# pminervini/hyperopt

Hardware: AMD Instinct MI355X
Metric: EI candidates scored/sec (x components) (higher is better)
Workload: dtype f64 (log-sum-exp: fp64 accumulation, fp32 exp2 of the shifted term, its argument from an fp32 block-local quadratic (mode 3); quantized: fp64 erf); 1 GPU; config 4: 100-D uniform space, 1e4-trial history, 1e7 candidates/suggest (lpdf roofline stress); parallelism=single

## Files before the change

hyperopt_amd/_engine.py:

```python
from __future__ import annotations

import ctypes as C
import os
import threading

import numpy as np

_HERE = os.path.dirname(os.path.abspath(__file__))
LIB_PATH = os.environ.get('TPE_ENGINE_LIB', os.path.join(_HERE, 'libtpe_engine.so'))

TPE_OK = 0
TPE_E_INVALID = -1
TPE_E_BOUNDS = -2
TPE_E_NEGATIVE = -3
TPE_E_NOMEM = -4
TPE_E_HIP = -5
TPE_E_NODEVICE = -6
TPE_E_INDEX = -7

GMM, LGMM, CAT = 0, 1, 2
HAS_LOW, HAS_HIGH, HAS_Q, PCHOICE = 1, 2, 4, 8
OBS_IDENT, OBS_LOG, OBS_LOG_CLIP_EXPLOW, OBS_LOG_CLIP_EPS = 0, 1, 2, 3
KIND_NAMES = ('lse_gmm', 'lse_lgmm', 'erf_gmm', 'erf_lgmm', 'categorical')

EXPORTS = (
    'tpe_version', 'tpe_device_count', 'tpe_create', 'tpe_destroy', 'tpe_last_error',
    'tpe_synchronize', 'tpe_split', 'tpe_parzen_fit', 'tpe_categorical_posterior',
    'tpe_lpdf', 'tpe_score', 'tpe_sample', 'tpe_plan_create', 'tpe_plan_destroy',
    'tpe_plan_num_levels', 'tpe_plan_set_history', 'tpe_plan_fit', 'tpe_plan_get_mixture',
    'tpe_plan_get_table',
    'tpe_plan_suggest', 'tpe_plan_suggest_shard', 'tpe_plan_merge', 'tpe_plan_score_candidates', 'tpe_plan_last_stats',
    'tpe_plan_profile', 'tpe_plan_profile_read', 'tpe_microbench', 'tpe_plan_get_results',
    'tpe_plan_results_device', 'tpe_plan_census', 'tpe_plan_fit_suggest',
    'tpe_plan_set_lattice', 'tpe_plan_update_history', 'tpe_plan_set_prune',
    'tpe_plan_sample_prior', 'tpe_plan_score_candidates_sorted', 'tpe_plan_census_n',
    'tpe_plan_tie_counts', 'tpe_plan_tab_wmax', 'tpe_plan_anneal', 'tpe_plan_anneal_trace',
    'tpe_plan_set_anneal_order', 'tpe_plan_tab_bound', 'tpe_plan_tab_hot',
    'tpe_plan_tab_panels', 'tpe_plan_tab_cert', 'tpe_plan_tie_list',
    'tpe_plan_cand_dump', 'tpe_plan_draw_screen_stats', 'tpe_plan_score_points',
    'tpe_plan_sample_points', 'tpe_plan_topk_points', 'tpe_plan_gather_points',
    'tpe_plan_joint_fit', 'tpe_plan_joint_get_mixture', 'tpe_plan_joint_score_points',
    'tpe_plan_joint_sides', 'tpe_plan_joint_sample_points', 'tpe_math_probe',
    'tpe_plan_group_info', 'tpe_plan_group_fit', 'tpe_plan_group_get_mixture',
    'tpe_plan_group_score_points', 'tpe_plan_group_sides', 'tpe_plan_group_sample_points',
    'tpe_plan_group_batch_points',
    'tpe_plan_set_objectives', 'tpe_plan_pareto_get', 'tpe_plan_pareto_shape',
    'tpe_plan_set_hv', 'tpe_plan_hv_get',
)

BATCH_MAX = 1024
MAX_OBJ = 8

SHARD_ALIGN = 8192


class EngineUnavailable(RuntimeError):
    """The HIP engine library or an MI355X (gfx950) device is not available."""


class EngineError(RuntimeError):
    pass


class TpeHp(C.Structure):
    _fields_ = [('family', C.c_int32), ('flags', C.c_uint32), ('obs_transform', C.c_int32),
                ('upper', C.c_int32), ('prior_mu', C.c_double), ('prior_sigma', C.c_double),
                ('low', C.c_double), ('high', C.c_double), ('q', C.c_double),
                ('cond_begin', C.c_int32), ('cond_count', C.c_int32),
                ('pprior_begin', C.c_int64)]


class TpeSpace(C.Structure):
    _fields_ = [('n_hp', C.c_int32), ('hp', C.POINTER(TpeHp)), ('n_cond', C.c_int32),
                ('cond_parent', C.POINTER(C.c_int32)), ('cond_branch', C.POINTER(C.c_int32)),
                ('n_pprior', C.c_int64), ('pprior', C.POINTER(C.c_double))]


RESULT_DTYPE = np.dtype([('score', '<f8'), ('value', '<f8'), ('index', '<i8'),
                         ('active', '<i4'), ('pad', '<i4')])
ANNEAL_TRACE_DTYPE = np.dtype([('row', '<i4'), ('rank', '<i4'), ('u', '<f8', (4,))])

_D = C.POINTER(C.c_double)
_lib = None
_lib_lock = threading.Lock()


def _share_hip_runtime():
    if os.environ.get('TPE_ENGINE_HIP_RUNTIME', '') == 'system':
        return
    import importlib.util
    try:
        spec = importlib.util.find_spec('torch')
    except (ImportError, ValueError):
        spec = None
    if spec is None or not spec.origin:
        return
    hip = os.path.join(os.path.dirname(spec.origin), 'lib', 'libamdhip64.so')
    if os.path.exists(hip):
        C.CDLL(hip, mode=C.RTLD_GLOBAL)


def load_library(path: str = LIB_PATH):
    global _lib
    with _lib_lock:
        if _lib is not None:
            return _lib
        if not os.path.exists(path):
            raise EngineUnavailable(
                'libtpe_engine.so not found at %s: build it with `make -C '
                'hyperopt_amd/csrc` or __graft_entry__.build()' % path)
        _share_hip_runtime()
        lib = C.CDLL(path)
        vp, i32, i64, u32, u64, dbl = C.c_void_p, C.c_int32, C.c_int64, C.c_uint32, C.c_uint64, C.c_double
        sig = {
            'tpe_version': (C.c_char_p, []),
            'tpe_device_count': (C.c_int, [C.POINTER(i32)]),
            'tpe_create': (C.c_int, [i32, C.POINTER(vp)]),
            'tpe_destroy': (C.c_int, [vp]),
            'tpe_last_error': (C.c_char_p, [vp]),
            'tpe_synchronize': (C.c_int, [vp]),
            'tpe_split': (C.c_int, [vp, _D, i64, dbl, i32, C.POINTER(C.c_uint8)]),
            'tpe_parzen_fit': (C.c_int, [vp, _D, i64, dbl, dbl, dbl, i32, _D, _D, _D]),
            'tpe_categorical_posterior': (C.c_int, [vp, C.POINTER(i64), i64, i32, dbl, _D, i32, _D]),
            'tpe_lpdf': (C.c_int, [vp, i32, _D, i64, _D, _D, _D, i64, dbl, dbl, dbl, u32, _D]),
            'tpe_score': (C.c_int, [vp, i32, _D, i64, _D, _D, _D, i64, _D, _D, _D, i64,
                                    dbl, dbl, dbl, u32, _D, _D, C.POINTER(i64), _D]),
            'tpe_sample': (C.c_int, [vp, i32, _D, _D, _D, i64, dbl, dbl, dbl, u32, u64, u64,
                                     i64, i64, _D]),
            'tpe_plan_create': (C.c_int, [vp, C.POINTER(TpeSpace), i64, C.POINTER(vp)]),
            'tpe_plan_destroy': (C.c_int, [vp]),
            'tpe_plan_num_levels': (C.c_int, [vp, C.POINTER(i32)]),
            'tpe_plan_set_history': (C.c_int, [vp, vp, vp, vp, i64, i32, vp]),
            'tpe_plan_update_history': (C.c_int, [vp, i64, i64, i64, vp, vp, i64, i64, vp, i32,
                                                  vp]),
            'tpe_plan_fit': (C.c_int, [vp, dbl, i32, dbl, i32, vp]),
            'tpe_plan_get_mixture': (C.c_int, [vp, i32, i32, _D, _D, _D, i64, C.POINTER(i64)]),
            'tpe_plan_get_table': (C.c_int, [vp, i32, i32, i32, vp, i64, C.POINTER(i64)]),
            'tpe_plan_suggest': (C.c_int, [vp, C.POINTER(u64), i64, i64, i64, i32, vp, i32, vp]),
            'tpe_plan_suggest_shard': (C.c_int, [vp, C.POINTER(u64), i64, i64, i64, i64, i32, vp,
                                                 i32, vp]),
            'tpe_plan_fit_suggest': (C.c_int, [vp, dbl, i32, dbl, i32, C.POINTER(u64), i64, i64,
                                               vp, i32, vp]),
            'tpe_plan_merge': (C.c_int, [vp, vp, i32, i32, vp, i32, vp]),
            'tpe_plan_score_candidates': (C.c_int, [vp, i32, _D, i64, _D, _D, C.POINTER(i64), _D]),
            'tpe_plan_score_candidates_sorted': (C.c_int, [vp, i32, i32, _D, i64, _D, _D,
                                                           C.POINTER(i64), _D]),
            'tpe_plan_score_points': (C.c_int, [vp, vp, i64, i64, vp, vp, vp, i32, vp]),
            'tpe_plan_sample_points': (C.c_int, [vp, u64, i64, i64, i64, vp, vp, vp, vp, i32, vp]),
            'tpe_plan_topk_points': (C.c_int, [vp, vp, vp, i64, i32, vp, i32, vp]),
            'tpe_plan_joint_fit': (C.c_int, [vp, vp]),
            'tpe_plan_joint_get_mixture': (C.c_int, [vp, i32, i32, _D, _D, _D, vp, i64,
                                                     C.POINTER(i64)]),
            'tpe_plan_joint_score_points': (C.c_int, [vp, vp, i64, i64, vp, vp, vp, vp, i32, vp]),
            'tpe_plan_joint_sides': (C.c_int, [vp, vp, vp, i64]),
            'tpe_plan_joint_sample_points': (C.c_int, [vp, u64, i64, i64, i64, vp, vp, vp, vp, vp,
                                                       vp, i32, vp]),
            'tpe_plan_group_info': (C.c_int, [vp, vp, C.POINTER(i32)]),
            'tpe_plan_group_fit': (C.c_int, [vp, vp]),
            'tpe_plan_group_get_mixture': (C.c_int, [vp, i32, i32, i32, _D, _D, _D, vp, i64,
                                                     C.POINTER(i64)]),
            'tpe_plan_group_score_points': (C.c_int, [vp, vp, i64, i64, vp, vp, vp, i32, vp]),
            'tpe_plan_group_sides': (C.c_int, [vp, i32, vp, vp, i64]),
            'tpe_plan_group_sample_points': (C.c_int, [vp, u64, i64, i64, i64, vp, vp, vp, vp, vp,
                                                       i32, vp]),
            'tpe_plan_group_batch_points': (C.c_int, [vp, vp, i64, i64, vp, i32, vp, vp, vp, i32,
                                                      vp]),
            'tpe_plan_gather_points': (C.c_int, [vp, vp, i64, vp, i32, vp, i32, vp]),
            'tpe_plan_set_objectives': (C.c_int, [vp, vp, i32, i64, i64, i64, i32, vp]),
            'tpe_plan_pareto_get': (C.c_int, [vp, vp, vp, vp, i64]),
            'tpe_plan_pareto_shape': (C.c_int, [vp, i64, i32, i64, C.POINTER(i64)]),
            'tpe_plan_set_hv': (C.c_int, [vp, i32, vp, i32, i32, i32, C.c_uint64, i32]),
            'tpe_plan_hv_get': (C.c_int, [vp, vp, vp, vp, C.POINTER(i32), i32]),
            'tpe_plan_last_stats': (C.c_int, [vp, _D, _D]),
            'tpe_plan_profile': (C.c_int, [vp, i32]),
            'tpe_plan_profile_read': (C.c_int, [vp, i32, _D, C.POINTER(i64), _D]),
            'tpe_microbench': (C.c_int, [vp, i32, _D]),
            'tpe_math_probe': (C.c_int, [vp, i32, _D, i64, _D]),
            'tpe_plan_get_results': (C.c_int, [vp, vp, i32, vp]),
            'tpe_plan_results_device': (vp, [vp]),
            'tpe_plan_census': (C.c_int, [vp, i32, C.POINTER(i64)]),
            'tpe_plan_census_n': (C.c_int, [vp, i32, C.POINTER(i64), i32]),
            'tpe_plan_tie_counts': (C.c_int, [vp, i32, vp]),
            'tpe_plan_tab_wmax': (C.c_int, [vp, i32, vp]),
            'tpe_plan_tab_bound': (C.c_int, [vp, i32, vp]),
            'tpe_plan_tab_hot': (C.c_int, [vp, i32, vp]),
            'tpe_plan_tab_panels': (C.c_int, [vp, i32, i32, vp, vp, vp, vp]),
            'tpe_plan_tab_cert': (C.c_int, [vp, i32, i32, vp]),
            'tpe_plan_tie_list': (C.c_int, [vp, i32, i32, vp]),
            'tpe_plan_cand_dump': (C.c_int64, [vp, i32, i32, vp, vp]),
            'tpe_plan_draw_screen_stats': (C.c_int, [vp, vp]),
            'tpe_plan_set_lattice': (C.c_int, [vp, i32]),
            'tpe_plan_set_prune': (C.c_int, [vp, i32]),
            'tpe_plan_sample_prior': (C.c_int, [vp, C.POINTER(u64), i64, vp, i32, vp]),
            'tpe_plan_anneal': (C.c_int, [vp, dbl, dbl, C.POINTER(u64), i64, vp, i32, vp]),
            'tpe_plan_anneal_trace': (C.c_int, [vp, i32, vp]),
            'tpe_plan_set_anneal_order': (C.c_int, [vp, C.POINTER(i32), i32]),
        }
        for name, (res, args) in sig.items():
            fn = getattr(lib, name)
            fn.restype = res
            fn.argtypes = args
        _lib = lib
        return lib


def _seeds(seeds):
    seeds = [int(x) & (2 ** 64 - 1) for x in np.atleast_1d(np.asarray(seeds, dtype=object))]
    return np.fromiter(seeds, dtype=np.uint64, count=len(seeds))


def _dp(a):
    return None if a is None else a.ctypes.data_as(_D)


def _f64(a):
    return np.ascontiguousarray(a, dtype=np.float64)


class Engine(object):

    def __init__(self, device: int = 0):
        self.lib = load_library()
        n = C.c_int32(0)
        self.lib.tpe_device_count(C.byref(n))
        if n.value <= 0:
            raise EngineUnavailable('no HIP device visible (TPE engine needs an MI355X)')
        h = C.c_void_p()
        rc = self.lib.tpe_create(int(device), C.byref(h))
        if rc != TPE_OK:
            raise EngineUnavailable('tpe_create(%d) failed (%d): not a gfx950 device?' % (device, rc))
        self.h = h
        self.device = device
        self.lock = threading.RLock()

    def close(self):
        if getattr(self, 'h', None):
            self.lib.tpe_destroy(self.h)
            self.h = None

    def __del__(self):
        try:
            self.close()
        except Exception:
            pass

    def check(self, rc):
        if rc == TPE_OK:
            return
        msg = (self.lib.tpe_last_error(self.h) or b'').decode()
        if rc == TPE_E_BOUNDS:
            raise ValueError('low >= high', msg)
        if rc == TPE_E_NEGATIVE:
            raise ValueError('negative arg to lognormal_cdf', msg)
        if rc == TPE_E_INDEX:
            raise IndexError(msg)
        if rc == TPE_E_INVALID:
            raise ValueError(msg)
        raise EngineError('TPE engine error %d: %s' % (rc, msg))

    def synchronize(self):
        with self.lock:
            self.check(self.lib.tpe_synchronize(self.h))

    def microbench(self, which):
        r = C.c_double(0)
        with self.lock:
            self.check(self.lib.tpe_microbench(self.h, int(which), C.byref(r)))
        return r.value

    def math_probe(self, which, x):
        xa = _f64(x)
        xs = xa.ravel()
        out = np.empty(xs.size)
# ... 741 lines not shown
        with e.lock:
            e.check(e.lib.tpe_plan_census_n(self.p, int(bool(enable)), out, int(n)))
        return tuple(int(v) for v in out[:n])

    def tie_counts(self, n_suggest):
        e = self.engine
        out = np.empty((int(n_suggest), self.n_hp), dtype=np.int32)
        with e.lock:
            e.check(e.lib.tpe_plan_tie_counts(self.p, int(n_suggest), out.ctypes.data))
        return out

    def tab_wmax(self, n_suggest):
        e = self.engine
        with e.lock:
            w = e.lib.tpe_plan_tab_wmax(self.p, int(n_suggest), None)
            e.check(min(w, 0))
            out = np.empty((int(n_suggest), self.n_hp, w), dtype=np.float64)
            e.check(e.lib.tpe_plan_tab_wmax(self.p, int(n_suggest), out.ctypes.data))
        return out

    def tab_bound(self, hp):
        e = self.engine
        with e.lock:
            n = e.lib.tpe_plan_tab_bound(self.p, int(hp), None)
            e.check(min(n, 0))
            out = np.empty(n, dtype=np.float64)
            e.check(e.lib.tpe_plan_tab_bound(self.p, int(hp), out.ctypes.data))
        return out

    def tab_panels(self, hp, side):
        e = self.engine
        y_lo, inv_w, ncert = C.c_double(), C.c_double(), C.c_int32()
        buf = np.zeros((64, 144), dtype=np.uint8)
        with e.lock:
            n = e.lib.tpe_plan_tab_panels(self.p, int(hp), int(side), C.addressof(y_lo),
                                          C.addressof(inv_w), C.addressof(ncert), buf.ctypes.data)
            e.check(min(n, 0))
        return dict(y_lo=y_lo.value, inv_w=inv_w.value, P=int(n), ncert=int(ncert.value),
                    panels=buf[:n].copy())

    def tab_cert(self, hp, side):
        e = self.engine
        out = np.zeros((64, 3), dtype=np.float64)
        with e.lock:
            n = e.lib.tpe_plan_tab_cert(self.p, int(hp), int(side), out.ctypes.data)
            e.check(min(n, 0))
        return out[:n].copy()

    def tie_list(self, s, hp):
        e = self.engine
        with e.lock:
            n = e.lib.tpe_plan_tie_list(self.p, int(s), int(hp), None)
            e.check(min(n, 0))
            out = np.empty(n, dtype=np.int32)
            if n:
                e.check(min(e.lib.tpe_plan_tie_list(self.p, int(s), int(hp), out.ctypes.data), 0))
        return out

    def tab_hot(self, n_suggest):
        e = self.engine
        out = np.empty((int(n_suggest), self.n_hp, 18), dtype=np.float64)
        with e.lock:
            e.check(e.lib.tpe_plan_tab_hot(self.p, int(n_suggest), out.ctypes.data))
        return out

    def cand_dump(self, s, hp):
        e = self.engine
        with e.lock:
            n = e.lib.tpe_plan_cand_dump(self.p, int(s), int(hp), None, None)
            e.check(int(min(n, 0)))
            vals = np.empty(n, dtype=np.float64)
            pos = np.empty(n, dtype=np.int32)
            e.check(int(min(e.lib.tpe_plan_cand_dump(self.p, int(s), int(hp), vals.ctypes.data,
                                                     pos.ctypes.data), 0)))
        return vals, pos

    def draw_screen_stats(self):
        e = self.engine
        out = np.zeros(3, dtype=np.int64)
        with e.lock:
            e.check(e.lib.tpe_plan_draw_screen_stats(self.p, out.ctypes.data))
        return int(out[0]), int(out[1]), int(out[2])

    def last_stats(self):
        e = self.engine
        ms, pairs = C.c_double(0), C.c_double(0)
        with e.lock:
            e.check(e.lib.tpe_plan_last_stats(self.p, C.byref(ms), C.byref(pairs)))
        return ms.value, pairs.value


_default = {}
_default_lock = threading.Lock()


def default_engine(device: int | None = None) -> Engine:
    if device is None:
        device = int(os.environ.get('LOCAL_RANK', '0'))
    with _default_lock:
        eng = _default.get(device)
        if eng is None:
            eng = Engine(device)
            _default[device] = eng
        return eng
```

hyperopt_amd/csrc/tpe_engine.hip:

```cpp
#include <hip/hip_runtime.h>

#include <algorithm>
#include <cmath>
#include <cstdlib>
#include <cstdio>
#include <cstring>
#include <string>
#include <vector>

#include "tpe_anneal.hpp"
#include "tpe_group_plan.hpp"
#include "tpe_internal.hpp"
#include "tpe_level_plan.hpp"
#include "tpe_pareto_plan.hpp"
#include "tpe_hv_plan.hpp"
#include "tpe_switches.hpp"

using namespace tpe;
static_assert(sizeof(AnnealTrace) == sizeof(tpe_anneal_trace), "layout");

struct tpe_engine {
  int32_t device = 0;
  hipStream_t stream = nullptr;
  static constexpr int kAux = 4;
  hipStream_t aux[kAux] = {};
  std::string err;
  tpe_plan *op = nullptr;
};

struct tpe_plan : PlanShape {
  tpe_engine *eng = nullptr;
  int32_t P = 0;
  int64_t ncap = 0;
  int32_t last_nb = -1;
  std::vector<double> pprior;
  std::vector<int32_t> level_off;
  tpe_hp *d_hps = nullptr;
  int32_t *d_cp = nullptr, *d_cb = nullptr, *d_level_hps = nullptr, *d_all_hps = nullptr;
  int32_t *d_level_off = nullptr;
  double *d_pprior = nullptr;
  double *d_losses = nullptr, *d_vals = nullptr;
  uint8_t *d_active = nullptr, *d_below = nullptr;
  double *d_mw = nullptr, *d_mmu = nullptr, *d_msig = nullptr, *d_scratch = nullptr;
  unsigned char *d_sortbuf = nullptr;
  int64_t scap = 0;
  MixInfo *d_info = nullptr;
  Coef *d_coef = nullptr;
  Coef32 *d_coef32 = nullptr;
  CoefM *d_coefm = nullptr;
  CoefM8 *d_coefm8 = nullptr;
  float4 *d_coefe = nullptr;
  CoefM8 *d_coefmh = nullptr;
  TabHdr *d_tab_hdr = nullptr;
  TabPanel *d_tab = nullptr;
  double *d_tab_max = nullptr;
  double *d_tab_wmax = nullptr;
  int32_t *d_tie_list = nullptr;
  int32_t *d_tie_cnt = nullptr;
  int32_t tab_pstride = 0;
  double *d_tab_bound = nullptr;
  double *d_tab_terms = nullptr;
  double *d_tab_cert = nullptr;
  TabHot *d_tab_hot = nullptr;
  DrawZone *d_draw_zone = nullptr;
  unsigned long long *d_screen_stats = nullptr;
  bool tab_built = false;
  bool graph_tab = false;
  int64_t n = 0;
  int64_t s_cap = 0;
  Partial *d_results = nullptr;
  tpe_result *h_results = nullptr;
  size_t h_results_cap = 0;
  uint64_t *h_flag = nullptr;
  uint64_t seq = 0;
  bool pub_fired = false;
  uint64_t *d_seeds = nullptr;
  Partial *d_partial = nullptr;
  size_t partial_cap = 0;
  unsigned long long *d_census = nullptr;
  bool census = false;
  uint32_t *d_ticket = nullptr;
  std::vector<uint64_t> h_seeds;
  bool has_erf = false;
  LatInfo *d_lat_info = nullptr;
  double2 *d_lat = nullptr;
  bool lattice_on = true;
  int32_t prune_mode = 3;
  hipEvent_t ev_fork = nullptr, ev_join[8] = {};
  double *d_ext = nullptr, *d_lb = nullptr, *d_la = nullptr;
  size_t ext_cap = 0;
  double *d_pt_vals = nullptr, *d_pt_terms = nullptr, *d_pt_total = nullptr;
  uint8_t *d_pt_act = nullptr;
  int32_t *d_pt_idx = nullptr;
  uint32_t *d_pt_count = nullptr;
  size_t pt_cap = 0;
  void *d_pt_tab = nullptr;
  void *d_tk = nullptr;
  int32_t *d_tk_idx = nullptr;
  double *d_cand = nullptr;
  int32_t *d_cpos = nullptr;
  size_t cand_cap = 0;
  std::vector<JointDim> jdims;
  std::vector<int32_t> jdim_of_hp;
  int32_t j_slots = 0;
  int64_t j_nopt = 0;
  bool joint_ok = false;
  int32_t jK[2] = {0, 0};
  double fit_pw = 1.0;
  int32_t fit_lf = 0;
  JointDim *d_jdims = nullptr;
  int32_t *d_jdim_of_hp = nullptr, *d_jrows = nullptr, *d_jcount = nullptr, *d_jcomp = nullptr;
  JointSide *d_jside = nullptr;
  uint64_t *d_jkeys = nullptr;
  double *d_jw = nullptr, *d_jcw = nullptr, *d_jcmu = nullptr, *d_jcsig = nullptr;
  double *d_jtab = nullptr, *d_joptlog = nullptr, *d_jpick = nullptr, *d_joptcdf = nullptr;
  size_t joptcdf_cap = 0;
  void *d_jdraw = nullptr;
  double *d_jsides = nullptr, *d_jjoint = nullptr;
  size_t jpt_cap = 0;
  int64_t jpt_m = 0;
  GroupPartition gpart;
  GroupLayout glay;
  bool group_ready = false, group_ok = false;
  int32_t gkb_max = 0;
  JointDim *d_gdims = nullptr;
  GroupDesc *d_ggroups = nullptr;
  int32_t *d_gdim_of_hp = nullptr, *d_ggroup_of_hp = nullptr, *d_grows = nullptr;
  int32_t *d_gcount = nullptr, *d_gcomp = nullptr;
  JointSide *d_gside = nullptr;
  uint64_t *d_gkeys = nullptr;
  double *d_gw = nullptr, *d_gcw = nullptr, *d_gcmu = nullptr, *d_gcsig = nullptr;
  double *d_gtab = nullptr, *d_goptlog = nullptr, *d_gpick = nullptr, *d_goptcdf = nullptr;
  size_t goptcdf_cap = 0;
  void *d_gdraw = nullptr;
  double *d_gsides = nullptr, *d_gjoint = nullptr;
  size_t gpt_cap = 0;
  int64_t gpt_m = 0;
  double *d_bt_ja = nullptr, *d_bt_score = nullptr, *d_bt_gain = nullptr, *d_bt_trace = nullptr;
  uint8_t *d_bt_gact = nullptr, *d_bt_state = nullptr;
  void *d_bt_slot = nullptr, *d_bt_rec = nullptr;
  int32_t *d_bt_idx = nullptr;
  size_t bt_cap = 0, bt_trace_cap = 0;
  int64_t bt_m = -1;
  hipEvent_t ev0 = nullptr, ev1 = nullptr;
  struct Prof {
    std::vector<hipEvent_t> a, b;
    std::vector<double> pairs;
    int64_t n = 0;
  };
  Prof prof[KIND_CAT + 1];
  int32_t prof_cap = 0;
  bool timed = false;
  bool evs = false;
  int64_t last_ncand = 0, last_nsug = 0;
  int32_t last_level = -1;
  int64_t dump_cn = 0, dump_sstride = 0, dump_nsug = 0;
  int32_t dump_level = -1;
  struct StepKey {
    double prior_weight = 0;
    int32_t lf = 0;
    void *stream = nullptr;
    StepShape shape;
    bool operator==(const StepKey &o) const {
      return prior_weight == o.prior_weight && lf == o.lf && stream == o.stream &&
             shape == o.shape;
    }
  };
  StepKey graph_key, pending_key;
  bool graph_ok = false, pending = false;
  int32_t mom_w = 0;
  bool mom_h = false;
// ... 31 lines not shown
  bool hv_last_exact = false;
  hipGraph_t graph = nullptr;
  hipGraphExec_t graph_exec = nullptr;
  std::vector<hipGraphNode_t> fit_nodes, draw_nodes;
  std::vector<hipKernelNodeParams> fit_params, draw_params;
  std::vector<FitArgs> fit_args0;
  std::vector<ScoreArgs> draw_args0;
};

namespace {

#define CKH(expr)                                                        \
  do {                                                                   \
    hipError_t e_ = (expr);                                              \
    if (e_ != hipSuccess) {                                              \
      return fail(h, TPE_E_HIP, std::string(#expr) + ": " + hipGetErrorString(e_)); \
    }                                                                    \
  } while (0)

int fail(tpe_engine *h, int code, const std::string &msg) {
  if (h) h->err = msg;
  return code;
}

template <typename T>
hipError_t dalloc(T **p, size_t count) {
  *p = nullptr;
  if (count == 0) count = 1;
  return hipMalloc((void **)p, count * sizeof(T));
}

void dfree(void *p) {
  if (p) (void)hipFree(p);
}

void graph_reset(tpe_plan *p) {
  if (p->graph_exec) (void)hipGraphExecDestroy(p->graph_exec);
  if (p->graph) (void)hipGraphDestroy(p->graph);
  p->graph_exec = nullptr;
  p->graph = nullptr;
  p->graph_ok = p->pending = false;
  p->fit_nodes.clear(); p->draw_nodes.clear();
  p->fit_params.clear(); p->draw_params.clear();
  p->fit_args0.clear(); p->draw_args0.clear();
}

hipStream_t pick_stream(tpe_engine *h, void *s) {
  return s ? (hipStream_t)s : h->stream;
}

void plan_free_buffers(tpe_plan *p) {
  void *bufs[] = {p->d_an_keys, p->d_an_idx, p->d_an_T, p->d_an_hporder, p->d_an_trace,
                  p->d_hps, p->d_cp, p->d_cb, p->d_level_hps, p->d_all_hps, p->d_pprior,
                  p->d_level_off,
                  p->d_losses, p->d_vals, p->d_active, p->d_below, p->d_mw, p->d_mmu,
                  p->d_msig, p->d_scratch, p->d_info, p->d_coef, p->d_results, p->d_seeds,
                  p->d_partial, p->d_ext, p->d_lb, p->d_la, p->d_cand, p->d_cpos,
                  p->d_ticket, p->d_sortbuf, p->d_census, p->d_lat_info, p->d_lat, p->d_coef32, p->d_coefm,
                  p->d_coefm8, p->d_coefe, p->d_coefmh, p->d_tab_hdr, p->d_tab,
                  p->d_tab_max, p->d_tab_wmax, p->d_tie_list, p->d_tie_cnt, p->d_tab_bound,
                  p->d_tab_terms, p->d_tab_cert,
                  p->d_tab_hot, p->d_draw_zone, p->d_screen_stats, p->d_pt_vals, p->d_pt_terms,
                  p->d_pt_total, p->d_pt_act, p->d_pt_idx, p->d_pt_count, p->d_pt_tab, p->d_tk,
                  p->d_tk_idx, p->d_jdims, p->d_jdim_of_hp, p->d_jrows, p->d_jcount, p->d_jcomp,
                  p->d_jside, p->d_jkeys, p->d_jw, p->d_jcw, p->d_jcmu, p->d_jcsig, p->d_jtab,
                  p->d_joptlog, p->d_jpick, p->d_joptcdf, p->d_jdraw, p->d_jsides, p->d_jjoint,
                  p->d_gdims, p->d_ggroups, p->d_gdim_of_hp, p->d_ggroup_of_hp, p->d_grows,
                  p->d_gcount, p->d_gcomp, p->d_gside, p->d_gkeys, p->d_gw, p->d_gcw, p->d_gcmu,
                  p->d_gcsig, p->d_gtab, p->d_goptlog, p->d_gpick, p->d_goptcdf, p->d_gdraw,
                  p->d_gsides, p->d_gjoint, p->d_bt_ja, p->d_bt_score, p->d_bt_gain,
                  p->d_bt_trace, p->d_bt_gact, p->d_bt_state, p->d_bt_slot, p->d_bt_rec,
                  p->d_bt_idx, p->d_obj, p->d_pcount, p->d_hv_i32, p->d_hv_f64, p->d_hv_alive,
                  p->d_hv_u};
  for (void *b : bufs) dfree(b);
  if (p->h_results) (void)hipHostFree(p->h_results);
  p->h_results = nullptr;
  p->h_results_cap = 0;
  if (p->h_flag) (void)hipHostFree(p->h_flag);
  p->h_flag = nullptr;
  if (p->ev0) (void)hipEventDestroy(p->ev0);
  if (p->ev1) (void)hipEventDestroy(p->ev1);
  if (p->ev_fork) (void)hipEventDestroy(p->ev_fork);
  for (auto e : p->ev_join) if (e) (void)hipEventDestroy(e);
  for (auto &pr : p->prof) {
    for (auto e : pr.a) (void)hipEventDestroy(e);
    for (auto e : pr.b) (void)hipEventDestroy(e);
    pr.a.clear(); pr.b.clear(); pr.pairs.clear(); pr.n = 0;
  }
}

int validate_space(tpe_engine *h, const tpe_space *sp) {
  if (!sp || sp->n_hp <= 0 || !sp->hp) return fail(h, TPE_E_INVALID, "empty space");
  for (int i = 0; i < sp->n_hp; ++i) {
    const tpe_hp &x = sp->hp[i];
    if (x.family < TPE_GMM || x.family > TPE_CAT)
      return fail(h, TPE_E_INVALID, "hp " + std::to_string(i) + ": bad family");
    if (x.family == TPE_CAT && x.upper <= 0)
      return fail(h, TPE_E_INVALID, "hp " + std::to_string(i) + ": categorical upper <= 0");
    if (x.family != TPE_CAT) {
      const bool hl = x.flags & TPE_HAS_LOW, hh = x.flags & TPE_HAS_HIGH;
      if (hl != hh)
        return fail(h, TPE_E_INVALID, "hp " + std::to_string(i) + ": one-sided truncation");
      if (hl && !(x.low < x.high))
        return fail(h, TPE_E_BOUNDS, "low >= high");
      if (!(x.prior_sigma > 0))
        return fail(h, TPE_E_INVALID, "hp " + std::to_string(i) + ": prior_sigma <= 0");
    }
    if (x.cond_count < 0 || x.cond_begin < 0 || x.cond_begin + x.cond_count > sp->n_cond)
      return fail(h, TPE_E_INVALID, "hp " + std::to_string(i) + ": bad condition range");
    for (int c = 0; c < x.cond_count; ++c) {
      const int par = sp->cond_parent[x.cond_begin + c];
      if (par < 0 || par >= sp->n_hp || par == i)
        return fail(h, TPE_E_INVALID, "hp " + std::to_string(i) + ": bad condition parent");
    }
    if ((x.flags & TPE_PCHOICE) &&
        (x.pprior_begin < 0 || x.pprior_begin + x.upper > sp->n_pprior))
      return fail(h, TPE_E_INVALID, "hp " + std::to_string(i) + ": bad pchoice prior");
  }
  return TPE_OK;
}

LatInfo lattice_of(const tpe_hp &x) {
  LatInfo L{0, 0, 0, 0};
  const int k = score_kind(x);
  if (k != KIND_ERF_G && k != KIND_ERF_L) return L;
  if (!(x.flags & TPE_HAS_LOW) || !(x.flags & TPE_HAS_HIGH) || !(x.q > 0.0)) return L;
  double lo = x.low, hi = x.high;
  if (k == KIND_ERF_L) {
    lo = std::exp(lo);
    hi = std::exp(hi);
  }
  const double a = std::rint(lo / x.q) - 2.0, b = std::rint(hi / x.q) + 2.0;
  if (!(std::fabs(a) < 1e15 && std::fabs(b) < 1e15) || b - a + 1.0 > (double)kLatMaxR)
    return L;
  L.j0 = (int64_t)a;
  L.R = (int32_t)(b - a + 1.0);
  return L;
}

int compute_levels(tpe_engine *h, tpe_plan *p) {
  std::vector<int> lev(p->P, -1);
  for (int iter = 0; iter <= p->P; ++iter) {
    bool changed = false;
    for (int i = 0; i < p->P; ++i) {
      const tpe_hp &x = p->hps[i];
      int l = 0;
      bool ready = true;
      for (int c = 0; c < x.cond_count; ++c) {
        const int par = p->cond_parent[x.cond_begin + c];
        if (lev[par] < 0) { ready = false; break; }
        l = std::max(l, lev[par] + 1);
      }
      if (ready && lev[i] != l) { lev[i] = l; changed = true; }
    }
    if (!changed) break;
  }
  int nl = 0;
  for (int i = 0; i < p->P; ++i) {
    if (lev[i] < 0 || lev[i] > p->P) return fail(h, TPE_E_INVALID, "cyclic conditions");
    nl = std::max(nl, lev[i] + 1);
  }
  p->levels.assign(nl, {});
  for (int lat : {1, 0})
    for (int kind : {KIND_ERF_L, KIND_ERF_G})
      for (int i = 0; i < p->P; ++i)
        if (score_kind(p->hps[i]) == kind && (lattice_of(p->hps[i]).R > 0) == (lat == 1))
// ... 10 lines not shown
int plan_build(tpe_engine *h, const tpe_space *sp, int64_t max_trials, tpe_plan *p) {
  int rc = validate_space(h, sp);
  if (rc) return rc;
  if (max_trials < 0) return fail(h, TPE_E_INVALID, "max_trials < 0");
  p->eng = h;
  p->P = sp->n_hp;

  p->hps.assign(sp->hp, sp->hp + sp->n_hp);
  p->cond_parent.assign(sp->cond_parent, sp->cond_parent + sp->n_cond);
  p->cond_branch.assign(sp->cond_branch, sp->cond_branch + sp->n_cond);
  p->pprior.assign(sp->pprior, sp->pprior + sp->n_pprior);
  rc = compute_levels(h, p);
  if (rc) return rc;
  p->ncap = std::max<int64_t>(max_trials, 1);
  int64_t kcap = p->ncap + 1;
  for (const auto &x : p->hps)
    if (x.family == TPE_CAT) kcap = std::max<int64_t>(kcap, x.upper);
  kcap = (kcap + kCoefBlock - 1) / kCoefBlock * kCoefBlock;
  p->kcap = kcap;
  for (const auto &x : p->hps) {
    const int k = score_kind(x);
    if (k == KIND_ERF_G || k == KIND_ERF_L) p->has_erf = true;
  }
  const int64_t slots = 2 * (int64_t)p->P;
  p->lat.assign(p->P, LatInfo{0, 0, 0, 0});
  int64_t lat_total = 0;
  for (int i = 0; i < p->P; ++i) {
    p->lat[i] = lattice_of(p->hps[i]);
    p->lat[i].off = lat_total;
    lat_total += p->lat[i].R;
  }
  CKH(hipSetDevice(h->device));
  CKH(dalloc(&p->d_lat_info, p->P));
  CKH(dalloc(&p->d_lat, std::max<int64_t>(1, lat_total)));
  CKH(dalloc(&p->d_hps, p->P));
  CKH(dalloc(&p->d_cp, p->cond_parent.size()));
  CKH(dalloc(&p->d_cb, p->cond_branch.size()));
  CKH(dalloc(&p->d_pprior, p->pprior.size()));
  CKH(dalloc(&p->d_level_hps, p->P));
  CKH(dalloc(&p->d_all_hps, p->P));
  CKH(dalloc(&p->d_level_off, p->level_off.size()));
  CKH(dalloc(&p->d_losses, p->ncap));
  CKH(dalloc(&p->d_vals, (size_t)p->ncap * p->P));
  CKH(dalloc(&p->d_active, (size_t)p->ncap * p->P));
  CKH(dalloc(&p->d_below, p->ncap));
  CKH(dalloc(&p->d_mw, (size_t)slots * kcap));
  CKH(dalloc(&p->d_mmu, (size_t)slots * kcap));
  CKH(dalloc(&p->d_msig, (size_t)slots * kcap));
  CKH(dalloc(&p->d_scratch, (size_t)slots * kcap));
  p->scap = p->ncap + 1;
  CKH(dalloc(&p->d_sortbuf, (size_t)slots * 16 * p->scap));
  CKH(dalloc(&p->d_info, slots));
  CKH(dalloc(&p->d_census, kCensus));
  CKH(hipMemset(p->d_census, 0, kCensus * sizeof(unsigned long long)));
  CKH(dalloc(&p->d_coef, (size_t)slots * kcap));
  CKH(dalloc(&p->d_coef32, (size_t)slots * (kcap / kCoefBlock)));
  CKH(dalloc(&p->d_coefm, (size_t)slots * mom_stride(kcap)));
  CKH(dalloc(&p->d_coefm8, (size_t)slots * (kcap / kCoefBlock)));
  CKH(dalloc(&p->d_coefe, (size_t)slots * (kcap / kCoefBlock)));
  CKH(dalloc(&p->d_coefmh, (size_t)slots * mom_stride(kcap)));
  CKH(dalloc(&p->d_tab_hdr, (size_t)slots));
  CKH(hipMemset(p->d_tab_hdr, 0, (size_t)slots * sizeof(TabHdr)));
  CKH(dalloc(&p->d_tab, (size_t)slots * kTabMaxPanels));
  CKH(dalloc(&p->d_tab_bound, (size_t)p->P * kBndCells));
  if (switches().table_lean) CKH(dalloc(&p->d_tab_terms, table_terms_doubles(p->P, kcap)));
  p->act_frac.assign(p->P, 1.0);
  for (const auto &lv : p->levels)
    for (int i : lv) {
      const tpe_hp &x = p->hps[i];
      if (x.cond_count == 0) continue;
      double f = 0.0;
      for (int c = 0; c < x.cond_count; ++c) {
        const int par = p->cond_parent[x.cond_begin + c];
        const tpe_hp &y = p->hps[par];
        f += p->act_frac[par] / (y.family == TPE_CAT ? std::max(1, (int)y.upper) : 1);
      }
      p->act_frac[i] = std::min(1.0, f);
    }
  p->finish();
  CKH(hipEventCreate(&p->ev0));
  CKH(hipEventCreate(&p->ev1));
  CKH(hipEventCreateWithFlags(&p->ev_fork, hipEventDisableTiming));
  for (auto &e : p->ev_join) CKH(hipEventCreateWithFlags(&e, hipEventDisableTiming));
  std::vector<int32_t> lh;
  for (auto &l : p->levels) lh.insert(lh.end(), l.begin(), l.end());
  std::vector<int32_t> all(p->P);
  for (int i = 0; i < p->P; ++i) all[i] = i;
  hipStream_t st = h->stream;
  CKH(hipMemcpyAsync(p->d_hps, p->hps.data(), p->P * sizeof(tpe_hp), hipMemcpyHostToDevice, st));
  CKH(hipMemcpyAsync(p->d_lat_info, p->lat.data(), p->P * sizeof(LatInfo), hipMemcpyHostToDevice,
                     st));
  if (!p->cond_parent.empty()) {
    CKH(hipMemcpyAsync(p->d_cp, p->cond_parent.data(), p->cond_parent.size() * 4, hipMemcpyHostToDevice, st));
    CKH(hipMemcpyAsync(p->d_cb, p->cond_branch.data(), p->cond_branch.size() * 4, hipMemcpyHostToDevice, st));
  }
  if (!p->pprior.empty())
    CKH(hipMemcpyAsync(p->d_pprior, p->pprior.data(), p->pprior.size() * 8, hipMemcpyHostToDevice, st));
  CKH(hipMemcpyAsync(p->d_level_hps, lh.data(), lh.size() * 4, hipMemcpyHostToDevice, st));
  CKH(hipMemcpyAsync(p->d_all_hps, all.data(), all.size() * 4, hipMemcpyHostToDevice, st));
  CKH(hipMemcpyAsync(p->d_level_off, p->level_off.data(), p->level_off.size() * 4,
                     hipMemcpyHostToDevice, st));
  CKH(hipMemsetAsync(p->d_info, 0, slots * sizeof(MixInfo), st));
  CKH(hipStreamSynchronize(st));
  return TPE_OK;
}

int ensure_suggest_state(tpe_engine *h, tpe_plan *p, int64_t n_sug, size_t partials) {
  if (n_sug > p->s_cap || partials > p->partial_cap) graph_reset(p);
  if (n_sug > p->s_cap) {
    dfree(p->d_results);
    dfree(p->d_seeds);
    dfree(p->d_ticket);
    p->d_results = nullptr;
    p->d_seeds = nullptr;
    p->d_ticket = nullptr;
    CKH(dalloc(&p->d_results, (size_t)n_sug * p->P));
    CKH(dalloc(&p->d_seeds, n_sug));
    CKH(dalloc(&p->d_ticket, (size_t)n_sug * p->P + 1));
    CKH(hipMemset(p->d_ticket, 0, ((size_t)n_sug * p->P + 1) * sizeof(uint32_t)));
    dfree(p->d_tab_max);
    p->d_tab_max = nullptr;
    CKH(dalloc(&p->d_tab_max, (size_t)n_sug * p->P));
    dfree(p->d_tie_cnt);
    p->d_tie_cnt = nullptr;
    CKH(dalloc(&p->d_tie_cnt, (size_t)n_sug * p->P));
    CKH(hipMemset(p->d_tie_cnt, 0xff, (size_t)n_sug * p->P * sizeof(int32_t)));
    dfree(p->d_tab_hot);
    p->d_tab_hot = nullptr;
    CKH(dalloc(&p->d_tab_hot, (size_t)n_sug * p->P));
    dfree(p->d_draw_zone);
    p->d_draw_zone = nullptr;
    CKH(dalloc(&p->d_draw_zone, (size_t)n_sug * p->P));
    if (!p->d_screen_stats) {
      CKH(dalloc(&p->d_screen_stats, 2));
      CKH(hipMemset(p->d_screen_stats, 0, 2 * sizeof(unsigned long long)));
    }
    p->s_cap = n_sug;
  }
  if (partials > p->partial_cap) {
    dfree(p->d_partial);
    p->d_partial = nullptr;
    CKH(dalloc(&p->d_partial, partials));
    dfree(p->d_tab_wmax);
    p->d_tab_wmax = nullptr;
    CKH(dalloc(&p->d_tab_wmax, partials * 8));
    CKH(hipMemset(p->d_tab_wmax, 0xff, partials * 8 * sizeof(double)));
    dfree(p->d_tie_list);
    p->d_tie_list = nullptr;
    CKH(dalloc(&p->d_tie_list, partials * 8));
    p->partial_cap = partials;
  }
  return TPE_OK;
}

int ensure_ext(tpe_engine *h, tpe_plan *p, size_t n) {
  if (n > p->ext_cap) {
    dfree(p->d_ext); dfree(p->d_lb); dfree(p->d_la);
    p->d_ext = p->d_lb = p->d_la = nullptr;
    CKH(dalloc(&p->d_ext, n));
    CKH(dalloc(&p->d_lb, n));
    CKH(dalloc(&p->d_la, n));
    p->ext_cap = n;
  }
  return TPE_OK;
}

// ... 113 lines not shown
  a.n_below = n_below;
  a.lf = lf;
  a.prior_weight = prior_weight;
  a.pprior = p->d_pprior;
  a.mw = p->d_mw;
  a.mmu = p->d_mmu;
  a.msig = p->d_msig;
  a.info = p->d_info;
  a.coef = p->d_coef;
  a.coef32 = p->d_coef32;
  a.coefm = p->mom_w == 16 ? p->d_coefm : nullptr;
  a.coefm8 = p->mom_w == 8 ? p->d_coefm8 : nullptr;
  a.coefmh = p->mom_h ? p->d_coefmh : nullptr;
  a.coefe = p->d_coefe;
  a.kcap = p->kcap;
  a.ob = p->d_scratch;
  a.tmp = p->d_scratch;
  a.sortbuf = p->d_sortbuf;
  a.scap = p->scap;
  return a;
}

int flush_patch(tpe_engine *h, tpe_plan *p, hipStream_t st) {
  if (!p->has_pend) return TPE_OK;
  p->has_pend = false;
  CKH(launch_hist_patch(p->pend, p->d_vals, p->d_active, p->d_losses, st));
  return TPE_OK;
}
int fit_launch(tpe_engine *h, tpe_plan *p, const FitArgs &a, int32_t n_hp, hipStream_t st) {
  CKH(launch_fit(a, n_hp, st, p->has_pend ? &p->pend : nullptr));
  p->has_pend = false;
  return TPE_OK;
}

int table_build(tpe_engine *h, tpe_plan *p, hipStream_t st) {
  if (p->tab_built) return TPE_OK;
  CKH(launch_table_build(p->d_hps, p->P, p->d_info, p->d_coef, p->kcap, p->d_tab_hdr, p->d_tab,
                         p->census ? p->d_census : nullptr, st,
                         switches().table_prefilter ? p->d_tab_bound : nullptr, p->d_tab_terms,
                         p->d_tab_cert));
  p->tab_built = true;
  return TPE_OK;
}

int score_launch(tpe_engine *h, tpe_plan *p, ScoreArgs a, bool has_erf, int64_t cn,
                 hipStream_t sg, bool record, int classes = 7) {
  tpe_plan::Prof *pr = nullptr;
  if (record && p->prof_cap > 0) {
    pr = &p->prof[0];
    if (pr->n >= p->prof_cap) pr = nullptr;
  }
  if (pr) CKH(hipEventRecord(pr->a[pr->n], sg));
  if (a.tab_on == 1 && (classes & 1)) {
    const int rc = table_build(h, p, sg);
    if (rc) return rc;
    p->tab_pstride = a.pstride;
  }
  CKH(launch_score(a, has_erf, sg, switches().side_streams ? h->aux[1] : nullptr, p->ev_join[1],
                   p->ev_join[2], classes));
  if (pr) {
    CKH(hipEventRecord(pr->b[pr->n], sg));
    pr->pairs[pr->n] = (double)cn * (double)a.n_suggest;
    pr->n++;
  }
  return TPE_OK;
}

StepShape step_shape(const tpe_plan *p, int64_t n_sug, int64_t n_cand, int64_t cand_begin,
                     int64_t n_total, int32_t last_nb, const FitVariant &f) {
  StepShape s;
  s.n_sug = n_sug;
  s.n_cand = n_cand;
  s.cand_begin = cand_begin;
  s.n_total = n_total;
  s.below = below_class(last_nb >= 0 ? (int64_t)last_nb + 1 : p->kcap);
  s.fit = f;
  s.prune_mode = p->prune_mode;
  s.lattice_on = p->lattice_on;
  s.screen_run = step_screen_run(switches());
  s.screen_halves = step_screen_halves(switches());
  s.screen_tail = (int32_t)switches().draw_screen_tail;
  s.screen_pool = switches().draw_screen_pool;
  s.table_lean = switches().table_lean;
  return s;
}

int run_level(tpe_engine *h, tpe_plan *p, int level, const StepShape &s, hipStream_t st) {
  const LevelPlan lp = plan_level(*p, switches(), s, level);
  const int64_t n_sug = s.n_sug;
  const int32_t n_level = lp.n_level, n_lat = lp.n_lat;
  const int32_t *lvl = p->d_level_hps + p->level_off[level];
  if (lp.empty) {
    if (n_level > 0) CKH(launch_merge(lvl, n_level, (int32_t)n_sug, p->P, 0, nullptr, p->d_results, st));
    return TPE_OK;
  }
  ScoreArgs la = base_args(p, n_sug);
  la.level_hps = lvl;
  la.n_slots = n_level;
  la.slot_rows = lp.slot_rows;
  la.compact = lp.compact ? 1 : 0;
  auto lat_bracket = [&](hipStream_t sl, auto launch) -> int {
    tpe_plan::Prof *pr = nullptr;
    if (p->prof_cap > 0 && p->prof[1].n < p->prof_cap) pr = &p->prof[1];
    if (pr) CKH(hipEventRecord(pr->a[pr->n], sl));
    CKH(launch());
    if (pr) {
      CKH(hipEventRecord(pr->b[pr->n], sl));
      pr->pairs[pr->n] = (double)level;
      pr->n++;
    }
    return TPE_OK;
  };
  auto lattice = [&](hipStream_t sl) -> int {
    return lat_bracket(sl, [&] {
      return launch_lattice(la, p->levels[level].data(), p->hps.data(), p->lat.data(), n_lat,
                            p->d_lat, sl, lp.lat_rows);
    });
  };
  const bool lat_side = lp.lat == LatRun::Side;
  bool lat_pending = lp.lat == LatRun::Deferred;
  if (lp.lat == LatRun::InOrder || lat_side) {
    hipStream_t sl = st;
    if (lat_side) {
      sl = h->aux[0];
      CKH(hipEventRecord(p->ev_fork, st));
      CKH(hipStreamWaitEvent(sl, p->ev_fork, 0));
    }
    const int lrc = lattice(sl);
    if (lat_side) {
      const hipError_t e1 = hipEventRecord(p->ev_join[0], sl);
      if (lrc) {
        if (e1 == hipSuccess) (void)hipStreamWaitEvent(st, p->ev_join[0], 0);
        return lrc;
      }
      if (e1 != hipSuccess) return fail(h, TPE_E_HIP, "lattice side stream join event");
    } else if (lrc) {
      return lrc;
    }
  }
  bool joined = !lat_side;
  auto chunks = [&]() -> int {
  for (const ChunkPlan &c : lp.chunks) {
    const int64_t cn = c.cn;
    if (c.grid.pstride < 0) return fail(h, TPE_E_INVALID, "level slots not grouped by lpdf kind");
    int rc = ensure_suggest_state(h, p, n_sug, (size_t)n_sug * p->P * c.grid.pstride);
    if (rc) return rc;
    rc = ensure_cand(h, p, (size_t)std::max<int64_t>(1, n_sug * n_level * cn));
    if (rc) return rc;
    ScoreArgs a = base_args(p, n_sug);
    copy_groups(a, c.grid);
    a.compact = lp.compact ? 1 : 0;
    a.cand = p->d_cand;
    a.cand_sstride = (int64_t)n_level * cn;
    a.n_cand = cn;
    a.cand_begin = s.cand_begin + c.c0;
    a.accumulate = c.accumulate ? 1 : 0;
    a.level_hps = lvl;
    a.n_slots = n_level;
    a.slot_rows = lp.slot_rows;
    a.cand_slot0 = 0;
    for (int i = 0; i < kInlineSeeds && i < n_sug; ++i) a.seed_inline[i] = p->h_seeds[i];
    a.n_inline_seeds = (int32_t)std::min<int64_t>(n_sug, kInlineSeeds);
    a.lse_pos = c.lse_pos;
    a.sort_log2 = c.sort_log2;
    a.lookup_draw = c.lookup_draw;
    a.lse_prune = c.lse_prune;
    a.lse_shift_min = lp.lse_shift_min;
    a.lse_f32 = c.lse_f32;
    a.tab_on = c.tab_on;
    a.tab_pref = c.tab_pref ? 1 : 0;
    if (c.lk_fork) {
// ... 816 lines not shown
  if (mi.K > cap) return fail(h, TPE_E_INVALID, "capacity too small");
  if (w) CKH(hipMemcpy(w, p->d_mw + slot * p->kcap, mi.K * 8, hipMemcpyDeviceToHost));
  if (mu) CKH(hipMemcpy(mu, p->d_mmu + slot * p->kcap, mi.K * 8, hipMemcpyDeviceToHost));
  if (sigma) CKH(hipMemcpy(sigma, p->d_msig + slot * p->kcap, mi.K * 8, hipMemcpyDeviceToHost));
  return TPE_OK;
}

int tpe_plan_get_table(tpe_plan_t p, int32_t hp, int32_t side, int32_t which, void *out,
                       int64_t cap_bytes, int64_t *bytes) {
  if (!p || !bytes) return TPE_E_INVALID;
  tpe_engine *h = p->eng;
  if (hp < 0 || hp >= p->P || side < 0 || side > 1 || which < 0 || which > 4)
    return fail(h, TPE_E_INVALID, "bad hp/side/table");
  CKH(hipSetDevice(h->device));
  CKH(hipDeviceSynchronize());
  const int64_t slot = 2 * (int64_t)hp + side;
  const void *src = nullptr;
  if (which == 0) {
    *bytes = p->kcap * (int64_t)sizeof(Coef);
    src = p->d_coef + slot * p->kcap;
  } else if (which == 1) {
    *bytes = p->kcap / kCoefBlock * (int64_t)sizeof(Coef32);
    src = p->d_coef32 + slot * (p->kcap / kCoefBlock);
  } else if (which == 2) {
    *bytes = mom_stride(p->kcap) * (int64_t)sizeof(CoefM);
    src = p->d_coefm + slot * mom_stride(p->kcap);
  } else if (which == 3) {
    *bytes = p->kcap / kCoefBlock * (int64_t)sizeof(CoefM8);
    src = p->d_coefm8 + slot * (p->kcap / kCoefBlock);
  } else {
    *bytes = mom_stride(p->kcap) * (int64_t)sizeof(CoefM8);
    src = p->d_coefmh + slot * mom_stride(p->kcap);
  }
  if (!out) return TPE_OK;
  if (*bytes > cap_bytes) return fail(h, TPE_E_INVALID, "capacity too small");
  CKH(hipMemcpy(out, src, (size_t)*bytes, hipMemcpyDeviceToHost));
  return TPE_OK;
}

int tpe_plan_suggest(tpe_plan_t p, const uint64_t *seeds, int64_t n_sug, int64_t n_cand,
                     int64_t cand_begin, int32_t level, tpe_result *out, int32_t out_on_device,
                     void *stream) {
  return tpe_plan_suggest_shard(p, seeds, n_sug, cand_begin + n_cand, cand_begin, n_cand, level,
                                out, out_on_device, stream);
}

int tpe_plan_suggest_shard(tpe_plan_t p, const uint64_t *seeds, int64_t n_sug, int64_t n_total,
                           int64_t cand_begin, int64_t n_cand, int32_t level, tpe_result *out,
                           int32_t out_on_device, void *stream) {
  if (!p) return TPE_E_INVALID;
  tpe_engine *h = p->eng;
  if (n_sug <= 0 || n_cand < 0 || cand_begin < 0 || !seeds || n_total < cand_begin + n_cand)
    return fail(h, TPE_E_INVALID, "bad args");
  if (level >= (int32_t)p->levels.size()) return fail(h, TPE_E_INVALID, "bad level");
  CKH(hipSetDevice(h->device));
  hipStream_t st = pick_stream(h, stream);
  int rc = ensure_suggest_state(h, p, n_sug, 1);
  if (rc) return rc;
  p->h_seeds.assign(seeds, seeds + n_sug);
  if (n_sug > kInlineSeeds)
    CKH(hipMemcpyAsync(p->d_seeds, seeds, n_sug * 8, hipMemcpyHostToDevice, st));
  if (p->prof_cap > 0) CKH(hipEventRecord(p->ev0, st));
  const int l0 = level < 0 ? 0 : level;
  const int l1 = level < 0 ? (int)p->levels.size() : level + 1;
  const StepShape s = step_shape(p, n_sug, n_cand, cand_begin, n_total, p->last_nb,
                                 FitVariant{fit_small(p->n), p->mom_w, p->mom_h});
  for (int l = l0; l < l1; ++l) {
    rc = run_level(h, p, l, s, st);
    if (rc) return rc;
  }
  if (p->prof_cap > 0) CKH(hipEventRecord(p->ev1, st));
  p->timed = true;
  p->evs = p->prof_cap > 0;
  p->last_ncand = n_cand;
  p->last_nsug = n_sug;
  p->last_level = level;
  return copy_results(h, p, n_sug, out, out_on_device, st);
}

namespace {

int enqueue_step(tpe_engine *h, tpe_plan *p, int32_t nb, double prior_weight, int32_t lf,
                 const StepShape &s, hipStream_t st) {
  {
    const int rc = fit_launch(h, p, fit_args(p, nb, prior_weight, lf, s.fit), p->P, st);
    if (rc) return rc;
  }
  p->last_nb = nb;
  for (int l = 0; l < (int)p->levels.size(); ++l) {
    const int rc = run_level(h, p, l, s, st);
    if (rc) return rc;
  }
  return TPE_OK;
}

int capture_step(tpe_engine *h, tpe_plan *p, int32_t nb, double prior_weight, int32_t lf,
                 const StepShape &s, hipStream_t st) {
  graph_reset(p);
  CKH(hipStreamBeginCapture(st, hipStreamCaptureModeThreadLocal));
  const int rc = enqueue_step(h, p, nb, prior_weight, lf, s, st);
  hipGraph_t g = nullptr;
  const hipError_t ec = hipStreamEndCapture(st, &g);
  if (rc || ec != hipSuccess || !g) {
    if (g) (void)hipGraphDestroy(g);
    return rc ? rc : fail(h, TPE_E_HIP, "graph capture failed");
  }
  p->graph = g;
  p->graph_mom_w = p->mom_w;
  p->graph_mom_h = p->mom_h;
  p->graph_tab = p->tab_built;
  CKH(hipGraphInstantiate(&p->graph_exec, g, nullptr, nullptr, 0));
  size_t nn = 0;
  CKH(hipGraphGetNodes(g, nullptr, &nn));
  std::vector<hipGraphNode_t> nodes(nn);
  CKH(hipGraphGetNodes(g, nodes.data(), &nn));
  for (hipGraphNode_t nd : nodes) {
    hipGraphNodeType ty;
    CKH(hipGraphNodeGetType(nd, &ty));
    if (ty != hipGraphNodeTypeKernel) continue;
    hipKernelNodeParams kp{};
    CKH(hipGraphKernelNodeGetParams(nd, &kp));
    if (kp.func == fit_kernel_fn(true) || kp.func == fit_kernel_fn(false)) {
      p->fit_nodes.push_back(nd);
      p->fit_params.push_back(kp);
      p->fit_args0.push_back(*static_cast<const FitArgs *>(kp.kernelParams[0]));
    } else if (is_draw_kernel_fn(kp.func) || kp.func == lattice_draw_kernel_fn()) {
      p->draw_nodes.push_back(nd);
      p->draw_params.push_back(kp);
      p->draw_args0.push_back(*static_cast<const ScoreArgs *>(kp.kernelParams[0]));
    }
  }
  if (p->fit_nodes.size() != 1) {
    graph_reset(p);
    return fail(h, TPE_E_HIP, "graph capture: fit node not found");
  }
  p->graph_ok = true;
  return TPE_OK;
}

int launch_step(tpe_engine *h, tpe_plan *p, int32_t nb, const uint64_t *seeds, int64_t n_sug,
                hipStream_t st) {
  for (size_t i = 0; i < p->fit_nodes.size(); ++i) {
    FitArgs fa = p->fit_args0[i];
    fa.n = p->n;
    fa.n_below = nb;
    HistPatch none{};
    void *args[2] = {&fa, &none};
    hipKernelNodeParams kp = p->fit_params[i];
    kp.kernelParams = args;
    kp.extra = nullptr;
    CKH(hipGraphExecKernelNodeSetParams(p->graph_exec, p->fit_nodes[i], &kp));
  }
  for (size_t i = 0; i < p->draw_nodes.size(); ++i) {
    ScoreArgs da = p->draw_args0[i];
    for (int64_t j = 0; j < n_sug; ++j) da.seed_inline[j] = seeds[j];
    da.n_inline_seeds = (int32_t)n_sug;
    hipKernelNodeParams kp = p->draw_params[i];
    LatJobs jobs{};
    double2 *lat_out = nullptr;
    int32_t *pos_out = nullptr;
    const DrawZone *zones = nullptr;
    unsigned long long *stats = nullptr;
    int32_t run = 0;
    void *args[5] = {&da, &jobs, &lat_out, &stats, &run};
    if (kp.func == lattice_draw_kernel_fn()) {
      jobs = *static_cast<const LatJobs *>(kp.kernelParams[1]);
// ... 1410 lines not shown
  TabHdr th[2];
  CKH(hipMemcpyAsync(th, p->d_tab_hdr + 2 * (int64_t)hp, sizeof(th), hipMemcpyDeviceToHost,
                     h->stream));
  CKH(hipStreamSynchronize(h->stream));
  for (const TabHdr &t : th)
    if (!(t.P > 0 && t.ncert == (uint32_t)t.P))
      return fail(h, TPE_E_INVALID, "Chebyshev table not certified");
  CKH(hipMemcpy(out, p->d_tab_bound + (int64_t)hp * kBndCells, kBndCells * sizeof(double),
                hipMemcpyDeviceToHost));
  return TPE_OK;
}

static int tab_header(tpe_plan *p, int32_t hp, int32_t side, TabHdr *th) {
  tpe_engine *h = p->eng;
  if (hp < 0 || hp >= p->P || side < 0 || side > 1) return fail(h, TPE_E_INVALID, "bad args");
  if (!table_hp(p->hps[hp])) return fail(h, TPE_E_INVALID, "hp has no Chebyshev table");
  CKH(hipSetDevice(h->device));
  CKH(hipDeviceSynchronize());
  const int rc = table_build(h, p, h->stream);
  if (rc) return rc;
  CKH(hipMemcpyAsync(th, p->d_tab_hdr + 2 * (int64_t)hp + side, sizeof(*th), hipMemcpyDeviceToHost,
                     h->stream));
  CKH(hipStreamSynchronize(h->stream));
  if (th->P < 0 || th->P > kTabMaxPanels) return fail(h, TPE_E_HIP, "table header out of range");
  return TPE_OK;
}

int tpe_plan_tab_panels(tpe_plan_t p, int32_t hp, int32_t side, double *y_lo, double *inv_w,
                        int32_t *ncert, void *panels) {
  if (!p) return TPE_E_INVALID;
  tpe_engine *h = p->eng;
  TabHdr th;
  const int rc = tab_header(p, hp, side, &th);
  if (rc) return rc;
  if (y_lo) *y_lo = th.y_lo;
  if (inv_w) *inv_w = th.inv_w;
  if (ncert) *ncert = (int32_t)th.ncert;
  if (panels && th.P > 0)
    CKH(hipMemcpy(panels, p->d_tab + (2 * (int64_t)hp + side) * kTabMaxPanels,
                  (size_t)th.P * sizeof(TabPanel), hipMemcpyDeviceToHost));
  return th.P;
}

int tpe_plan_tab_cert(tpe_plan_t p, int32_t hp, int32_t side, double *out) {
  if (!p) return TPE_E_INVALID;
  tpe_engine *h = p->eng;
  if (!p->d_tab_cert) {
    CKH(hipSetDevice(h->device));
    CKH(hipDeviceSynchronize());
    graph_reset(p);
    const size_t n = (size_t)2 * p->P * kTabMaxPanels * 3;
    CKH(dalloc(&p->d_tab_cert, n));
    CKH(hipMemset(p->d_tab_cert, 0xff, n * sizeof(double)));
    p->tab_built = false;
  }
  TabHdr th;
  const int rc = tab_header(p, hp, side, &th);
  if (rc) return rc;
  if (out && th.P > 0)
    CKH(hipMemcpy(out, p->d_tab_cert + (2 * (int64_t)hp + side) * kTabMaxPanels * 3,
                  (size_t)th.P * 3 * sizeof(double), hipMemcpyDeviceToHost));
  return th.P;
}

int tpe_plan_tie_list(tpe_plan_t p, int32_t s, int32_t hp, int32_t *out) {
  if (!p) return TPE_E_INVALID;
  tpe_engine *h = p->eng;
  if (hp < 0 || hp >= p->P || s < 0 || s >= p->s_cap || p->tab_pstride <= 0 ||
      ((size_t)s * p->P + hp + 1) * p->tab_pstride > p->partial_cap)
    return fail(h, TPE_E_INVALID, "hp / suggestion not of the last launch that took the tables");
  CKH(hipSetDevice(h->device));
  CKH(hipDeviceSynchronize());
  int32_t n = 0;
  CKH(hipMemcpy(&n, p->d_tie_cnt + (int64_t)s * p->P + hp, sizeof(n), hipMemcpyDeviceToHost));
  const int64_t row = (int64_t)p->tab_pstride * 8;
  if (n < 0) return 0;
  if (n > row) return fail(h, TPE_E_HIP, "tie count out of range");
  if (out && n > 0)
    CKH(hipMemcpy(out, p->d_tie_list + ((int64_t)s * p->P + hp) * row, (size_t)n * sizeof(int32_t),
                  hipMemcpyDeviceToHost));
  return n;
}

int tpe_plan_draw_screen_stats(tpe_plan_t p, int64_t *out) {
  if (!p || !out) return TPE_E_INVALID;
  tpe_engine *h = p->eng;
  out[0] = out[1] = out[2] = 0;
  if (!p->d_screen_stats) return TPE_OK;
  CKH(hipSetDevice(h->device));
  CKH(hipDeviceSynchronize());
  unsigned long long v[2];
  CKH(hipMemcpy(v, p->d_screen_stats, sizeof(v), hipMemcpyDeviceToHost));
  CKH(hipMemset(p->d_screen_stats, 0, sizeof(v)));
  out[0] = (int64_t)(v[0] >> 40);
  out[1] = (int64_t)v[1];
  out[2] = (int64_t)(v[0] & ((1ull << 40) - 1));
  return TPE_OK;
}

int tpe_plan_tab_hot(tpe_plan_t p, int32_t n_suggest, double *out) {
  static_assert(sizeof(TabHot) == (2 + 2 * kHotIv) * sizeof(double), "y_lo, y_hi, lo[], hi[]");
  if (!p || !out || n_suggest < 0) return TPE_E_INVALID;
  tpe_engine *h = p->eng;
  if (n_suggest > p->s_cap) return fail(h, TPE_E_INVALID, "more suggestions than the last call's");
  CKH(hipSetDevice(h->device));
  CKH(hipDeviceSynchronize());
  if (n_suggest > 0)
    CKH(hipMemcpy(out, p->d_tab_hot, (size_t)n_suggest * p->P * sizeof(TabHot),
                  hipMemcpyDeviceToHost));
  return TPE_OK;
}

int tpe_plan_sample_prior(tpe_plan_t p, const uint64_t *seeds, int64_t n_sug, tpe_result *out,
                          int32_t out_on_device, void *stream) {
  if (!p) return TPE_E_INVALID;
  tpe_engine *h = p->eng;
  if (n_sug <= 0 || !seeds) return fail(h, TPE_E_INVALID, "bad args");
  CKH(hipSetDevice(h->device));
  hipStream_t st = pick_stream(h, stream);
  int rc = ensure_suggest_state(h, p, n_sug, 1);
  if (rc) return rc;
  CKH(hipMemcpyAsync(p->d_seeds, seeds, n_sug * 8, hipMemcpyHostToDevice, st));
  PriorArgs a{};
  a.hps = p->d_hps;
  a.n_hp = p->P;
  a.n_levels = (int32_t)p->levels.size();
  a.level_hps = p->d_level_hps;
  a.level_off = p->d_level_off;
  a.cond_parent = p->d_cp;
  a.cond_branch = p->d_cb;
  a.pprior = p->d_pprior;
  a.seeds = p->d_seeds;
  a.results = p->d_results;
  CKH(launch_prior(a, (int32_t)n_sug, st));
  p->last_nsug = n_sug;
  if (!out_on_device) {
    rc = copy_results(h, p, n_sug, out, 0, st);
    if (rc) return rc;
    return TPE_OK;
  }
  return copy_results(h, p, n_sug, out, out_on_device, st);
}

int tpe_plan_set_anneal_order(tpe_plan_t p, const int32_t *hp_order, int32_t n_hp) {
  if (!p) return TPE_E_INVALID;
  tpe_engine *h = p->eng;
  if (!hp_order || n_hp != p->P) return fail(h, TPE_E_INVALID, "anneal order: one entry per hp");
  std::vector<int32_t> pos(p->P, -1);
  for (int k = 0; k < n_hp; ++k) {
    const int hp = hp_order[k];
    if (hp < 0 || hp >= p->P || pos[hp] >= 0)
      return fail(h, TPE_E_INVALID, "anneal order: not a permutation of the hps");
    pos[hp] = k;
  }
  for (int hp = 0; hp < p->P; ++hp) {
    const tpe_hp &x = p->hps[hp];
    for (int c = 0; c < x.cond_count; ++c)
      if (pos[p->cond_parent[x.cond_begin + c]] > pos[hp])
        return fail(h, TPE_E_INVALID, "anneal order: an hp before the choice that leads to it");
  }
  CKH(hipSetDevice(h->device));
  p->an_order = false;
  if (!p->d_an_hporder) CKH(dalloc(&p->d_an_hporder, p->P));
  CKH(hipDeviceSynchronize());
  CKH(hipMemcpy(p->d_an_hporder, hp_order, (size_t)n_hp * 4, hipMemcpyHostToDevice));
  p->an_order = true;
// ... 179 lines not shown
```

hyperopt_amd/csrc/tpe_fit.hip:

```cpp
#include <math.h>

#include "tpe_device.hpp"

#pragma clang fp contract(off)

namespace tpe {

#define NOINLINE __attribute__((noinline))

#ifdef TPE_STAMPS
__device__ unsigned long long g_stamps[512][48];
#define STAMP(ph)                                                             \
  do {                                                                        \
    if (threadIdx.x == 0 && blockIdx.z == 0)                                  \
      g_stamps[(2 * blockIdx.x + blockIdx.y) & 511][ph] = wall_clock64();     \
  } while (0)
#else
#define STAMP(ph) do {} while (0)
#endif

constexpr int kFitWaves = kFitThreads / 64;
constexpr int kSortCap = 10000;
constexpr int kMixLds = 4097;
constexpr int kMixStride = 4104;
// ... 863 lines not shown
  __syncthreads();
  uint32_t tot = 0, mine = 0;
#pragma unroll
  for (int w = 0; w < kFitWaves; ++w) {
    const uint32_t c = wc[w * kCatFastBins + lane];
    tot += c;
    mine += w < wv ? c : 0u;
  }
  const uint32_t start = wave_excl_scan_u32(tot);
  if (wv == 0 && lane < upper) {
    seg[2 * lane] = (int)start;
    seg[2 * lane + 1] = (int)(start + tot);
  }
  uint32_t run = start + mine;
  double *ws = reinterpret_cast<double *>(C.lds + kOffKeys);
  const LfRamp lr = lf_ramp(m, A.lf);
  const uint64_t lt = lane ? (~0ull >> (64 - lane)) : 0ull;
#pragma unroll
  for (int q = 0; q < kCatFastChunks; ++q) {
    if (q * 64 >= per) break;
    uint32_t rank = 0, inc = 0;
    for (int b = 0; b < upper; ++b) {
      const uint64_t bal = __ballot(kr[q] == b);
      if (kr[q] == b) rank = (uint32_t)__popcll(bal & lt);
      if (lane == b) inc = (uint32_t)__popcll(bal);
    }
    const uint32_t base = (uint32_t)__shfl((int)run, kr[q] < 0 ? 0 : kr[q], 64);
    if (kr[q] >= 0) ws[base + rank] = lf_weight(lr, (int64_t)(r0 + q * 64 + lane));
    run += inc;
  }
  __syncthreads();
  STAMP(41);
  categorical_tail(A, sm, H, slot, seg, ws);
}

__device__ __forceinline__ void categorical_tail(const FitArgs &A, FitShared &sm, const tpe_hp &H,
                                                 int64_t slot, const int *seg, const double *ws) {
  const int upper = H.upper;
  double *w = A.mw + slot * A.kcap, *mu = A.mmu + slot * A.kcap, *sg = A.msig + slot * A.kcap;
  for (int c = threadIdx.x; c < upper; c += blockDim.x) {
    double cnt = 0.0;
    const int r1 = seg[2 * c + 1];
    int r = seg[2 * c];
    for (; r + 8 <= r1; r += 8) {
      double wv[8];
#pragma unroll
      for (int u = 0; u < 8; ++u) wv[u] = ws[r + u];
#pragma unroll
      for (int u = 0; u < 8; ++u) cnt += wv[u];
    }
    for (; r < r1; ++r) cnt += ws[r];
    double pc;
    if (H.flags & TPE_PCHOICE)
      pc = cnt + (double)upper * (A.prior_weight * A.pprior[H.pprior_begin + c]);
    else
      pc = cnt + A.prior_weight;
    w[c] = pc;
  }
  __syncthreads();
  STAMP(5);
  const double tot = block_np_sum(w, upper, sm);
  for (int c = threadIdx.x; c < upper; c += blockDim.x) {
    w[c] = w[c] / tot;
    mu[c] = 0.0;
    sg[c] = 0.0;
  }
  __syncthreads();
  prep_slot(A.hps + slot / 2, slot, upper, w, mu, sg, A.info, A.coef, A.coef32, A.coefm, A.coefm8,
            A.coefe, A.kcap, A.tmp + slot * A.kcap, sm);
}

#ifndef TPE_FIT_REPS
#define TPE_FIT_REPS 1
#endif
template <bool SMALL>
__device__ __forceinline__ void fit_slot(const FitArgs &A, unsigned char *dyn_lds,
                                         FitShared &sm);

template <bool SMALL>
__global__ __launch_bounds__(kFitThreads) void k_fit(FitArgs A, HistPatch P) {
  extern __shared__ __attribute__((aligned(16))) unsigned char dyn_lds[];
  __shared__ FitShared sm;
  if (P.n_rows > 0 || P.n_loss > 0) {
    const int hp = blockIdx.x;
    double *vals = const_cast<double *>(A.vals);
    uint8_t *act = const_cast<uint8_t *>(A.active);
    double *losses = const_cast<double *>(A.losses);
    for (int r = threadIdx.x; r < (int)P.n_rows; r += blockDim.x) {
      vals[(int64_t)hp * P.ld + P.row0 + r] = P.vals[hp * (int)P.n_rows + r];
      act[(int64_t)hp * P.ld + P.row0 + r] = P.active[hp * (int)P.n_rows + r];
    }
    for (int i = threadIdx.x; i < (int)P.n_loss; i += blockDim.x) losses[P.loss0 + i] = P.losses[i];
    __threadfence_block();
    __syncthreads();
  }
  for (int rep = 0; rep < TPE_FIT_REPS; ++rep) {
    fit_slot<SMALL>(A, dyn_lds, sm);
    __syncthreads();
  }
}

template <bool SMALL>
__device__ __forceinline__ void fit_slot(const FitArgs &A, unsigned char *dyn_lds,
                                         FitShared &sm) {
  const int hp = blockIdx.x, side = blockIdx.y;
  const int64_t slot = 2 * (int64_t)hp + side;
  const tpe_hp H = A.hps[hp];
  FitCtx C;
  C.lds = dyn_lds;
  unsigned char *gsb = A.sortbuf + slot * 16 * A.scap;
  C.gkeys = reinterpret_cast<uint64_t *>(gsb);
  C.gpa = reinterpret_cast<uint32_t *>(gsb + 8 * A.scap);
  C.gpb = C.gpa + A.scap;
  STAMP(0);
#ifdef TPE_STAMPS
  const unsigned long long clk0 = clock64();
#endif
  const bool pre = SMALL || A.n <= kPreN;
  constexpr int PER = SMALL ? 1 : kGatherRows;
  const double *row = A.vals + (int64_t)hp * A.ld;
  const uint8_t *arow = A.active + (int64_t)hp * A.ld;
  double prv[PER];
  uint8_t pac[PER];
  if (pre) {
#pragma unroll
    for (int u = 0; u < PER; ++u) {
      const int64_t j = min<int64_t>((int64_t)u * kFitThreads + threadIdx.x, A.n - 1);
      pac[u] = j >= 0 ? arow[j] : 0;
      prv[u] = j >= 0 ? row[j] : 0.0;
    }
  }
  const Split t = compute_split<SMALL>(A, C, sm);
  __syncthreads();
  STAMP(1);

  const bool cat = H.family == TPE_CAT;
  double *ob = (SMALL || A.n <= kMergeMax)
                   ? reinterpret_cast<double *>(dyn_lds + kOffKeys + 8 * kMergeMax)
                   : A.ob + slot * A.kcap;
  uint64_t *lk = reinterpret_cast<uint64_t *>(dyn_lds + kOffKeys);
  const uint64_t *lkey = (SMALL || A.n <= kSortCap) ? lk : C.gkeys;
  int m = 0;
  const int lane = threadIdx.x & 63, wv = threadIdx.x >> 6;
  for (int64_t c0 = 0; c0 < A.n; c0 += PER * kFitThreads) {
    if (!pre) {
#pragma unroll
      for (int u = 0; u < PER; ++u) {
        const int64_t j = min<int64_t>(c0 + (int64_t)u * kFitThreads + threadIdx.x, A.n - 1);
        pac[u] = arow[j];
        prv[u] = row[j];
      }
    }
    uint32_t fm = 0u;
#pragma unroll
    for (int u = 0; u < PER; ++u) {
      const int64_t j = c0 + (int64_t)u * kFitThreads + threadIdx.x;
      const bool f = j < A.n && pac[u] && (is_below(t, lkey[j], (uint32_t)j) == (side == 0));
      fm |= f ? 1u << u : 0u;
      const uint64_t b = __ballot(f);
      if (lane == 0) sm.gcnt[u][wv] = (int)__popcll(b);
    }
    STAMP(35);
    __syncthreads();
    if (wv == 0) {
      constexpr int NE = PER * kFitWaves, E = (NE + 63) / 64;
      const int *gc = &sm.gcnt[0][0];
      int *gb = &sm.gbase[0][0];
      int c[E], loc = 0;
#pragma unroll
      for (int e = 0; e < E; ++e) {
        const int q = lane * E + e;
        c[e] = q < NE ? gc[q] : 0;
        loc += c[e];
      }
      int acc = wave_incl_scan(loc) - loc;
#pragma unroll
      for (int e = 0; e < E; ++e) {
        const int q = lane * E + e;
        if (q < NE) gb[q] = acc;
        acc += c[e];
      }
    }
    __syncthreads();
    STAMP(36);
#pragma unroll
    for (int u = 0; u < PER; ++u) {
      const bool f = (fm >> u) & 1u;
      const uint64_t b = __ballot(f);
// ... 151 lines not shown
```

hyperopt_amd/csrc/tpe_internal.hpp:

```cpp
#pragma once
#include <hip/hip_runtime.h>
#include <stdint.h>

#include "../../include/tpe_engine.h"

namespace tpe {

constexpr double kEPS = 1e-12;
constexpr int kFitThreads = 1024;
constexpr int kScoreThreads = 256;
constexpr int kMaxLeaves = 160;

enum { KIND_LSE_G = 0, KIND_LSE_L = 1, KIND_ERF_G = 2, KIND_ERF_L = 3, KIND_CAT = 4,
       KIND_LAT = 5, KIND_LSE_G1 = 6, KIND_LSE_L1 = 7, KIND_LSE_GW = 8, KIND_LSE_LW = 9,
       KIND_LSE_GW1 = 10, KIND_LSE_LW1 = 11 };
constexpr int64_t kWaveRowSplitMax = (int64_t)1 << 18;

__host__ __device__ constexpr bool kind_lse(int k) {
  return k == KIND_LSE_G || k == KIND_LSE_L || k == KIND_LSE_G1 || k == KIND_LSE_L1 ||
         k == KIND_LSE_GW || k == KIND_LSE_LW || k == KIND_LSE_GW1 || k == KIND_LSE_LW1;
}
__host__ __device__ constexpr bool kind_logn(int k) {
  return k == KIND_LSE_L || k == KIND_LSE_L1 || k == KIND_LSE_LW || k == KIND_LSE_LW1 ||
         k == KIND_ERF_L;
// ... 169 lines not shown
  const int32_t *cand_pos;
  double *out_lb, *out_la;
  Partial *results;
  Partial *partial;
  uint32_t *ticket;
  int64_t kcap;
  int64_t n_cand;
  int64_t cand_begin;
  int64_t cand_sstride;
  int32_t cand_slot0;
  int32_t pstride;
  int32_t n_hp;
  int32_t n_slots;
  int32_t n_suggest;
  int32_t n_groups;
  int32_t grp_kind[kMaxGroups];
  int32_t grp_slot0[kMaxGroups];
  int32_t grp_tiles[kMaxGroups];
  int32_t grp_block0[kMaxGroups + 1];
  int32_t grp_slots[kMaxGroups];
  int32_t compact;
  int32_t slot_rows;
  int32_t force_active;
  int32_t accumulate;
  unsigned long long *census;
  int32_t lse_pos;
  int32_t sort_log2;
  int32_t lse_prune;
  int32_t lse_shift_min;
  int32_t lse_f32;
  int32_t lse_mom;
  int32_t lse_momh;
  int32_t lookup_draw;
  int64_t lookup_seg;
  int32_t l2_warm;
  int32_t lse_tight;
  int32_t tile_draw;
  const LatInfo *lat_info;
  const double2 *lat;
  const TabHdr *tab_hdr;
  const TabPanel *tab;
  int32_t tab_on;
  double *tab_max;
  double *tab_wmax;
  int32_t *tie_list;
  int32_t *tie_cnt;
  double tab_tie;
  const double *tab_bound;
  TabHot *tab_hot;
  int32_t tab_pref;
  uint64_t *pub_dst;
  uint64_t *pub_flag;
  uint32_t *pub_ticket;
  uint64_t pub_seq;
  int32_t pub_words;
  int32_t pub_events;
};

struct FitArgs {
  const tpe_hp *hps;
  const double *vals;
  const uint8_t *active;
  const double *losses;
  int64_t n;
  int64_t ld;
  int32_t n_below;
  int32_t lf;
  int32_t pad0;
  double prior_weight;
  const double *pprior;
  double *mw, *mmu, *msig;
  MixInfo *info;
  Coef *coef;
  Coef32 *coef32;
  CoefM *coefm;
  CoefM8 *coefm8;
  CoefM8 *coefmh;
  float4 *coefe;
  int64_t kcap;
  double *ob;
  double *tmp;
  unsigned char *sortbuf;
  int64_t scap;
};

hipError_t launch_split(const FitArgs &a, uint8_t *below, hipStream_t st);
struct HistPatch;
hipError_t launch_fit(const FitArgs &a, int32_t n_hp, hipStream_t st,
                      const HistPatch *patch = nullptr);
bool fit_small(int64_t n);
const void *fit_kernel_fn(bool small);
bool is_draw_kernel_fn(const void *f);
bool is_sorted_draw_kernel_fn(const void *f);
bool is_prune_draw_kernel_fn(const void *f);
const void *lattice_draw_kernel_fn();
hipError_t launch_prep(const tpe_hp *hps, int32_t n_hp, const double *mw,
                       const double *mmu, const double *msig, MixInfo *info,
                       Coef *coef, Coef32 *coef32, CoefM *coefm, CoefM8 *coefm8,
                       float4 *coefe, int64_t kcap, double *scratch, hipStream_t st);
hipError_t launch_score(const ScoreArgs &a, bool has_erf, hipStream_t st,
                        hipStream_t side = nullptr, hipEvent_t ev_fork = nullptr,
                        hipEvent_t ev_join = nullptr, int classes = 7);
int score_classes(const ScoreArgs &a);
constexpr int kLatThreads = 256;
struct LatJob {
  tpe_hp H;
  LatInfo L;
  int32_t hp;
  int32_t pad;
};
constexpr int kLatJobs = 8;
struct LatJobs {
  LatJob job[kLatJobs];
  int32_t n_jobs;
  int32_t draw_gx;
  int32_t draw_blocks;
  int32_t compact;
  int32_t n_lat;
  int32_t pad[3];
};
constexpr int kFuseTab = 32;
hipError_t launch_lattice(const ScoreArgs &a, const int32_t *hps_of_level, const tpe_hp *hps,
                          const LatInfo *lat, int32_t n_lat, double2 *lat_out, hipStream_t st,
                          int32_t lat_rows);
hipError_t launch_lattice_draw(const ScoreArgs &a, const int32_t *hps_of_level, const tpe_hp *hps,
                               const LatInfo *lat, int32_t n_lat, double2 *lat_out,
                               hipStream_t st, int32_t lat_rows);
constexpr int kTabCap = 2048;
hipError_t launch_draw(const ScoreArgs &a, bool table, hipStream_t st);
constexpr int kSortedBlock = TPE_SHARD_ALIGN;
constexpr int kSortLog2Large = 13, kSortLog2Small = 12;
static_assert((1 << kSortLog2Large) == kSortedBlock, "largest sort block");
__host__ __device__ constexpr int sort_log2_for(int64_t n_total) {
  return n_total > kWaveRowSplitMax ? kSortLog2Large : kSortLog2Small;
}
hipError_t launch_draw_sorted(const ScoreArgs &a, bool small_table, bool fast, int32_t *pos_out,
                              hipStream_t st, int64_t max_blocks = INT64_MAX);
hipError_t launch_draw_pruned(const ScoreArgs &a, bool small_table, bool fast, int32_t *pos_out,
                              hipStream_t st);
constexpr int kZoneMax = 6;
constexpr int kZoneEdges = 2 * kZoneMax - 2;
constexpr double kScreenMargin = 1.6e-5;
constexpr int kGuideBitsMax = 10;
struct __attribute__((aligned(16))) DrawZone {
  int32_t nz;
  int32_t gbits;
  double gap_lo[kZoneMax - 1];
  double gap_hi[kZoneMax - 1];
  double thr[kFuseTab][kZoneEdges];
  uint64_t thrI[kFuseTab][kZoneEdges];
  uint64_t pickB[kFuseTab];
  uint16_t guide[1 << kGuideBitsMax];
  double tcdf[kFuseTab], tbase[kFuseTab], tmass[kFuseTab];
  unsigned char tmode[kFuseTab];
};
hipError_t launch_draw_zone(const ScoreArgs &a, DrawZone *zones, int32_t tiles, int32_t halves,
                            int32_t tail, double margin, int32_t guide_bits, hipStream_t st);
constexpr int kScreenRunMax = 16;
hipError_t launch_draw_screened(const ScoreArgs &a, int32_t *pos_out, const DrawZone *zones,
                                unsigned long long *stats, bool integer, int32_t run, bool pool,
                                hipStream_t st);
bool is_screen_draw_kernel_fn(const void *f);
bool is_screen_run_kernel_fn(const void *f);
hipError_t launch_table_pilot(const ScoreArgs &a, hipStream_t st);
static_assert(kSortedBlock == TPE_SHARD_ALIGN, "shard alignment is the sorted-draw block");
hipError_t launch_sort_ext(const ScoreArgs &a, const double *src, int32_t *pos_out,
                           hipStream_t st);
hipError_t launch_bucket(const ScoreArgs &a, int32_t slot_begin, int32_t *pos_out, hipStream_t st);
hipError_t launch_publish(const void *src, void *dst, size_t bytes, uint64_t *flag, uint64_t seq,
                          hipStream_t st);
hipError_t launch_merge(const int32_t *level_hps, int32_t n_slots,
                        int32_t n_suggest, int32_t n_hp, int32_t world,
                        const Partial *gathered, Partial *results,
                        hipStream_t st, Partial *out2 = nullptr);
hipError_t launch_sample(const tpe_hp *hp_dev, const double *mw,
                         const double *mmu, const double *msig,
                         const MixInfo *info, uint64_t seed, uint64_t stream,
                         int64_t offset, int64_t n, double *out,
                         hipStream_t st);

hipError_t launch_micro(int which, int blocks, int iters, double *sink, hipStream_t st);
hipError_t launch_math_probe(int which, const double *x, int64_t n, double *out, hipStream_t st);
constexpr int kTabTermDoubles = 4;
inline size_t table_terms_doubles(int32_t n_hp, int64_t kcap) {
  return (size_t)2 * n_hp * ((size_t)kcap * kTabTermDoubles + 1);
}
hipError_t launch_table_build(const tpe_hp *hps, int32_t n_hp, const MixInfo *info,
                              const Coef *coef, int64_t kcap, TabHdr *hdr, TabPanel *tab,
                              unsigned long long *census, hipStream_t st, double *bound = nullptr,
                              double *terms = nullptr, double *cert = nullptr);

constexpr int kPatchVals = 192;
constexpr int kPatchLoss = 16;
struct HistPatch {
  int64_t row0, n_rows, loss0, n_loss, ld;
  int32_t P;
  int32_t pad;
  double vals[kPatchVals];
  double losses[kPatchLoss];
  uint8_t active[kPatchVals];
};
hipError_t launch_hist_patch(const HistPatch &h, double *vals, uint8_t *active, double *losses,
                             hipStream_t st);

struct PriorArgs {
  const tpe_hp *hps;
  int32_t n_hp;
  int32_t n_levels;
  const int32_t *level_hps;
  const int32_t *level_off;
  const int32_t *cond_parent;
  const int32_t *cond_branch;
  const double *pprior;
  const uint64_t *seeds;
  Partial *results;
};
hipError_t launch_prior(const PriorArgs &a, int32_t n_suggest, hipStream_t st);

struct PointsArgs {
  const tpe_hp *hps;
  const int32_t *level_hps;
  const int32_t *cond_parent;
  const int32_t *cond_branch;
  const MixInfo *info;
  const Coef *coef;
  int64_t kcap;
  const double *vals;
  int64_t m, ld;
  uint8_t *active;
  double *terms;
  double *total;
  int64_t act_ld, term_ld;
  int32_t *idx;
  uint32_t *count;
  int32_t n_hp;
  int32_t pad;
};
hipError_t launch_points(const PointsArgs &a, hipStream_t st);
hipError_t launch_points_score(const PointsArgs &a, hipStream_t st);

template <int CAP> struct DrawTableT;
struct SampleArgs {
  PointsArgs P;
  double *out;
  const double *mw, *mmu, *msig;
  DrawTableT<kTabCap> *tab;
  uint64_t seed;
  int64_t begin;
};
size_t sample_tables_bytes(int32_t n_hp);
hipError_t launch_sample_points(const SampleArgs &s, hipStream_t st);

struct JointDim {
  int32_t hp;
  int32_t kind;
  int32_t slot;
  int32_t upper;
  int64_t opt_off;
};
__host__ __device__ constexpr int joint_slots(int kind) {
  return kind == KIND_CAT ? 4 : (kind == KIND_ERF_G || kind == KIND_ERF_L) ? 2 : 1;
}
constexpr int kJointFields = 3;
__host__ __device__ constexpr int64_t joint_stride(int32_t n_dim) {
  return (int64_t)kCoefBlock * (1 + kJointFields * (int64_t)n_dim);
}
struct JointSide {
  double tot;
  double a1;
};
struct JointFitArgs {
  const tpe_hp *hps;
  const JointDim *dims;
// ... 237 lines not shown
```

hyperopt_amd/csrc/tpe_kernels.hip:

```cpp
#include <math.h>

#include <algorithm>
#include <cstdlib>

#include "tpe_draw.hpp"
#include "tpe_tab_add.hpp"

namespace tpe {

constexpr int kSortMax = 8192;

constexpr int kDrawThreads = 256;
constexpr int kWideDrawThreads = 1024;
template <bool TAB>
__global__ __launch_bounds__(kDrawThreads) void k_draw(ScoreArgs A) {
  if constexpr (TAB) {
    __shared__ DrawTable T;
    draw_block<kTabCap>(A, blockIdx.x, blockIdx.y, blockIdx.z, T, (int64_t)gridDim.x * blockDim.x);
  } else {
    const int s = blockIdx.z;
    const int slot = row_slot(A, s, 0, A.n_slots, blockIdx.y);
    if (slot < 0) return;
    const int hp = A.level_hps[slot];
    const tpe_hp H = A.hps[hp];
// ... 526 lines not shown
    for (int j = 0; j < 4; ++j) v[j] = 1e-3 * (t + j);
    for (int i = 0; i < iters; ++i) {
#pragma unroll
      for (int j = 0; j < 4; ++j) v[j] = erf(v[j]) - 0.25;
    }
    double acc = 0.0;
#pragma unroll
    for (int j = 0; j < 4; ++j) acc += v[j];
    if (acc == 12345.0) sink[t] = acc;
  }
}


hipError_t launch_micro(int which, int blocks, int iters, double *sink, hipStream_t st) {
  switch (which) {
    case 0: k_micro<0><<<blocks, 256, 0, st>>>(iters, sink); break;
    case 1: k_micro<1><<<blocks, 256, 0, st>>>(iters, sink); break;
    case 3: k_micro<3><<<blocks, 256, 0, st>>>(iters, sink); break;
    case 4: k_micro<4><<<blocks, 256, 0, st>>>(iters, sink); break;
    case 5: k_micro<5><<<blocks, 256, 0, st>>>(iters, sink); break;
    case 6: k_micro<6><<<blocks, 256, 0, st>>>(iters, sink); break;
    case 7: k_micro<7><<<blocks, 256, 0, st>>>(iters, sink); break;
    case 8: k_micro<8><<<blocks, 256, 0, st>>>(iters, sink); break;
    case 9: k_micro<9><<<blocks, 256, 0, st>>>(iters, sink); break;
    default: k_micro<2><<<blocks, 256, 0, st>>>(iters, sink); break;
  }
  return hipGetLastError();
}

template <int WHICH>
__global__ __launch_bounds__(256) void k_math_probe(const double *__restrict__ x, int64_t n,
                                                    double *__restrict__ out) {
  const int64_t i = (int64_t)blockIdx.x * blockDim.x + threadIdx.x;
  if (i < n) {
    const double v = x[i];
    if constexpr (WHICH == 0) out[i] = fast_log(v);
    else if constexpr (WHICH == 1) out[i] = fast_log2(v);
    else if constexpr (WHICH == 2) out[i] = erfcinv_fast(v);
    else out[i] = erfc(v);
  }
}

hipError_t launch_math_probe(int which, const double *x, int64_t n, double *out, hipStream_t st) {
  if (n <= 0) return hipSuccess;
  const unsigned blocks = (unsigned)((n + 255) / 256);
  switch (which) {
    case 0: k_math_probe<0><<<blocks, 256, 0, st>>>(x, n, out); break;
    case 1: k_math_probe<1><<<blocks, 256, 0, st>>>(x, n, out); break;
    case 2: k_math_probe<2><<<blocks, 256, 0, st>>>(x, n, out); break;
    default: k_math_probe<3><<<blocks, 256, 0, st>>>(x, n, out); break;
  }
  return hipGetLastError();
}

bool is_draw_kernel_fn(const void *f) {
  return f == reinterpret_cast<const void *>(&k_draw<true>) ||
         f == reinterpret_cast<const void *>(&k_draw<false>) ||
         is_sorted_draw_kernel_fn(f);
}

bool is_sorted_draw_kernel_fn(const void *f) {
  return f == reinterpret_cast<const void *>(&k_draw_sorted<kFuseTab>) ||
         f == reinterpret_cast<const void *>(&k_draw_sorted<kTabCap>) ||
         f == reinterpret_cast<const void *>(&k_draw_sorted_fast<kFuseTab>) ||
         f == reinterpret_cast<const void *>(&k_draw_sorted_fast<kTabCap>) ||
         f == reinterpret_cast<const void *>(&k_draw_sorted_wide<kFuseTab>) ||
         f == reinterpret_cast<const void *>(&k_draw_sorted_wide<kTabCap>) ||
         f == reinterpret_cast<const void *>(&k_draw_sorted_wide_fast<kFuseTab>) ||
         f == reinterpret_cast<const void *>(&k_draw_sorted_wide_fast<kTabCap>) ||
         is_prune_draw_kernel_fn(f);
}

hipError_t launch_draw(const ScoreArgs &a, bool table, hipStream_t st) {
  if (a.n_slots <= 0 || a.n_suggest <= 0 || a.n_cand <= 0) return hipSuccess;
  const int64_t per = a.n_cand * a.slot_rows * a.n_suggest >= ((int64_t)1 << 22) ? 8 : 1;
  const unsigned gx = (unsigned)((a.n_cand + kDrawThreads * per - 1) / (kDrawThreads * per));
  const dim3 g(gx, (unsigned)a.slot_rows, a.n_suggest);
  if (table) k_draw<true><<<g, kDrawThreads, 0, st>>>(a);
  else k_draw<false><<<g, kDrawThreads, 0, st>>>(a);
  return hipGetLastError();
}

hipError_t launch_draw_sorted(const ScoreArgs &a, bool small_table, bool fast, int32_t *pos_out,
                              hipStream_t st, int64_t max_blocks) {
  if (a.n_slots <= 0 || a.n_suggest <= 0 || a.n_cand <= 0) return hipSuccess;
  const int64_t sbk = (int64_t)1 << a.sort_log2;
  const unsigned gx = (unsigned)std::min<int64_t>((a.n_cand + sbk - 1) / sbk, max_blocks);
  const dim3 g(gx, (unsigned)a.slot_rows, a.n_suggest);
  const bool wide = (int64_t)gx * a.slot_rows * a.n_suggest <= 2 * kNumCUs;
  if (wide) {
    if (fast) {
      if (small_table) k_draw_sorted_wide_fast<kFuseTab><<<g, kWideDrawThreads, 0, st>>>(a, pos_out);
      else k_draw_sorted_wide_fast<kTabCap><<<g, kWideDrawThreads, 0, st>>>(a, pos_out);
    } else {
      if (small_table) k_draw_sorted_wide<kFuseTab><<<g, kWideDrawThreads, 0, st>>>(a, pos_out);
      else k_draw_sorted_wide<kTabCap><<<g, kWideDrawThreads, 0, st>>>(a, pos_out);
    }
  } else if (fast) {
    if (small_table) k_draw_sorted_fast<kFuseTab><<<g, kSortThreads, 0, st>>>(a, pos_out);
    else k_draw_sorted_fast<kTabCap><<<g, kSortThreads, 0, st>>>(a, pos_out);
  } else if (small_table) {
    k_draw_sorted<kFuseTab><<<g, kSortThreads, 0, st>>>(a, pos_out);
  } else {
    k_draw_sorted<kTabCap><<<g, kSortThreads, 0, st>>>(a, pos_out);
  }
  return hipGetLastError();
}

hipError_t launch_sort_ext(const ScoreArgs &a, const double *src, int32_t *pos_out,
                           hipStream_t st) {
  if (a.n_slots <= 0 || a.n_suggest != 1 || a.n_cand <= 0) return hipSuccess;
  const int64_t sbk = (int64_t)1 << a.sort_log2;
  const unsigned gx = (unsigned)((a.n_cand + sbk - 1) / sbk);
  k_sort_ext<<<dim3(gx, a.n_slots, 1), kDrawThreads, 0, st>>>(a, src, pos_out);
  return hipGetLastError();
}

hipError_t launch_bucket(const ScoreArgs &a, int32_t slot_begin, int32_t *pos_out, hipStream_t st) {
  if (a.n_slots <= slot_begin || a.n_suggest <= 0 || a.n_cand <= 0) return hipSuccess;
  const unsigned gx = (unsigned)((a.n_cand + kSortMax - 1) / kSortMax);
  const unsigned rows = (unsigned)std::min(a.n_slots - slot_begin, a.slot_rows);
  k_bucket<<<dim3(gx, rows, a.n_suggest), 1024, (size_t)kSortMax * 9, st>>>(
      a, slot_begin, pos_out);
  return hipGetLastError();
}

__global__ __launch_bounds__(256) void k_publish(const uint64_t *__restrict__ src,
                                                 uint64_t *__restrict__ dst, int64_t n_words,
                                                 uint64_t *__restrict__ flag, uint64_t seq) {
  for (int64_t i = threadIdx.x; i < n_words; i += blockDim.x) dst[i] = src[i];
  __syncthreads();
  if (threadIdx.x == 0) {
    __builtin_amdgcn_fence(__ATOMIC_RELEASE, "");
    __hip_atomic_store(flag, seq, __ATOMIC_RELAXED, __HIP_MEMORY_SCOPE_SYSTEM);
  }
}

hipError_t launch_publish(const void *src, void *dst, size_t bytes, uint64_t *flag, uint64_t seq,
                          hipStream_t st) {
  k_publish<<<1, 256, 0, st>>>(static_cast<const uint64_t *>(src), static_cast<uint64_t *>(dst),
                               (int64_t)(bytes / 8), flag, seq);
  return hipGetLastError();
}

hipError_t launch_merge(const int32_t *level_hps, int32_t n_slots, int32_t n_suggest,
                        int32_t n_hp, int32_t world, const Partial *gathered,
                        Partial *results, hipStream_t st, Partial *out2) {
  if (n_slots <= 0 || n_suggest <= 0) return hipSuccess;
  k_merge<<<dim3(n_slots, n_suggest), 64, 0, st>>>(level_hps, n_slots, n_suggest, n_hp, world,
                                                   gathered, results, out2);
  return hipGetLastError();
}

hipError_t launch_sample(const tpe_hp *hp_dev, const double *mw, const double *mmu,
                         const double *msig, const MixInfo *info, uint64_t seed,
                         uint64_t stream, int64_t offset, int64_t n, double *out,
                         hipStream_t st) {
  if (n <= 0) return hipSuccess;
  const int64_t blocks = (n + 255) / 256;
  k_sample<<<(unsigned)blocks, 256, 0, st>>>(hp_dev, mw, mmu, msig, info, seed, (uint32_t)stream,
                                             offset, n, out);
  return hipGetLastError();
}

constexpr int kTabThreads = 256;
constexpr double kTabSkip = 64.0;

__device__ __forceinline__ void tab_merge(TabAcc &a, const TabAcc &b) {
  const double M = fmax(a.m, b.m);
  const double ms = M == -INFINITY ? 0.0 : M;
  a.s = ldexp(a.s, (int)fmax(a.m - ms, -2100.0)) + ldexp(b.s, (int)fmax(b.m - ms, -2100.0));
  a.m = M;
}
__device__ __forceinline__ TabAcc tab_wave_sum(TabAcc a) {
#pragma unroll
  for (int o = 32; o > 0; o >>= 1) {
    const TabAcc b{__shfl_xor(a.m, o, 64), __shfl_xor(a.s, o, 64)};
    tab_merge(a, b);
  }
  return a;
}

struct __attribute__((aligned(32))) TabTerm {
  double mu;
  double cc;
  double Ak;
  double ak;
};
constexpr double kTabL2E = 1.4426950408889634;
#pragma clang fp contract(off)
__device__ __forceinline__ TabTerm tab_term(double x, double y, double z) {
  TabTerm t;
  t.ak = -z;
  t.mu = y / (2.0 * t.ak);
  t.cc = __builtin_fma(t.ak * t.mu, t.mu, x);
  t.Ak = t.cc + 8.0 * log2(2.0 * t.ak / kTabL2E);
  return t;
}
__device__ __forceinline__ void tab_cert_terms(const TabTerm &t, double pl, double ph, double &te,
                                               double &tg) {
  const double d = fmax(0.0, fmax(pl - t.mu, t.mu - ph)), df = fmax(t.mu - pl, ph - t.mu);
  te = __builtin_fma(-((0.5 * t.ak) * d), d, t.Ak);
  tg = __builtin_fma(-(t.ak * df), df, t.cc);
}
#pragma clang fp contract(fast)

__global__ __launch_bounds__(kTabThreads) void k_table_terms(
    const tpe_hp *__restrict__ hps, const MixInfo *__restrict__ info,
    const Coef *__restrict__ coef, int64_t kcap, TabTerm *__restrict__ terms,
    double *__restrict__ a2s) {
  const int slot = blockIdx.y, tid = threadIdx.x, k = blockIdx.x * kTabThreads + tid;
  if (!table_hp(hps[slot >> 1])) return;
  const int K = info[slot].K;
  if (K < 1 || K > kcap) return;
  const double *__restrict__ cf = reinterpret_cast<const double *>(coef + (int64_t)slot * kcap);
  if (k < K)
    terms[(int64_t)slot * kcap + k] =
        tab_term(cf[coef_off(k, 0)], cf[coef_off(k, 1)], cf[coef_off(k, 2)]);
  if (blockIdx.x != 0) return;
  __shared__ double red[4];
  double a2 = 0.0;
  for (int k0 = tid; k0 < K; k0 += 4 * kTabThreads) {
    double z[4];
#pragma unroll
    for (int j = 0; j < 4; ++j) z[j] = cf[coef_off(min(k0 + j * kTabThreads, K - 1), 2)];
#pragma unroll
    for (int j = 0; j < 4; ++j) a2 = fmax(a2, -z[j]);
  }
#pragma unroll
  for (int o = 32; o > 0; o >>= 1) a2 = fmax(a2, __shfl_xor(a2, o, 64));
  if ((tid & 63) == 0) red[tid >> 6] = a2;
  __syncthreads();
  if (tid == 0) a2s[slot] = fmax(fmax(red[0], red[1]), fmax(red[2], red[3]));
}

template <bool LEAN>
__device__ __forceinline__ void table_build_body(
    const tpe_hp *__restrict__ hps, const MixInfo *__restrict__ info,
    const Coef *__restrict__ coef, int64_t kcap, TabHdr *__restrict__ hdr,
    TabPanel *__restrict__ tab, unsigned long long *__restrict__ census,
    const TabTerm *__restrict__ terms, const double *__restrict__ a2s,
    double *__restrict__ cert_out) {
  const int slot = blockIdx.y, p = blockIdx.x, tid = threadIdx.x;
  const tpe_hp H = hps[slot >> 1];
  if (!table_hp(H)) return;
  const MixInfo mi = info[slot];
  const int K = mi.K;
  if (K < 1 || K > kcap) return;
  const double *__restrict__ cf = reinterpret_cast<const double *>(coef + (int64_t)slot * kcap);
  __shared__ double red[4];
  __shared__ TabAcc acc[16][16];
  __shared__ TabAcc cert[2][4];
  __shared__ double fn[kTabNodes], cn[kTabNodes];
  __shared__ unsigned live_n;
  double a2 = 0.0;
  if constexpr (LEAN) {
    if (tid == 0) live_n = 0u;
    __syncthreads();
    a2 = a2s[slot];
  } else {
    for (int k = tid; k < K; k += kTabThreads) a2 = fmax(a2, -cf[coef_off(k, 2)]);
#pragma unroll
    for (int o = 32; o > 0; o >>= 1) a2 = fmax(a2, __shfl_xor(a2, o, 64));
    if ((tid & 63) == 0) red[tid >> 6] = a2;
    if (tid == 0) live_n = 0u;
    __syncthreads();
    a2 = fmax(fmax(red[0], red[1]), fmax(red[2], red[3]));
  }
  const double L2E = 1.4426950408889634;
  const double y_lo = H.low - H.prior_mu, y_hi = H.high - H.prior_mu;
  const double sig = sqrt(0.5 * L2E / a2);
  const double Pd = ceil((y_hi - y_lo) / (2.0 * sig));
  if (!(Pd >= 1.0 && Pd <= (double)kTabMaxPanels)) return;
  const int P = (int)Pd;
  if (p >= P) return;
  const double w = (y_hi - y_lo) / Pd, Hh = 0.5 * w;
  if (p == 0 && tid == 0) {
    hdr[slot].y_lo = y_lo;
    hdr[slot].inv_w = 1.0 / w;
    hdr[slot].P = P;
  }
  const double pl = y_lo + w * (double)p, ph = y_lo + w * (double)(p + 1), pc = pl + Hh;
  double thr = -INFINITY;
  if (mi.probe >= 0 && mi.probe < K) {
    const double x = cf[coef_off(mi.probe, 0)], y = cf[coef_off(mi.probe, 1)],
                 z = cf[coef_off(mi.probe, 2)];
    const double t0 = fma(z, pl * pl, fma(y, pl, x)), t1 = fma(z, ph * ph, fma(y, ph, x));
    const double tm = fmin(t0, t1);
    if (tm == tm) thr = tm - kTabSkip;
  }
  const int j = tid & 15, l = tid >> 4;
  const double yn = pc + Hh * cospi((double)(2 * j + 1) / 32.0), yn2 = yn * yn;
  TabAcc a{-INFINITY, 0.0};
  unsigned nlive = 0;
  const int nb = (K + kCoefBlock - 1) / kCoefBlock;
  for (int b = l; b < nb; b += 16) {
    const float4 e = reinterpret_cast<const float4 *>(cf)[(int64_t)b * 16 + 12];
    const double d = fmax(0.0, fmax((double)e.x - ph, pl - (double)e.y));
    const double bound = (double)e.z - (double)fabsf(e.w) * d * d;
    if (bound < thr) continue;
    const double *__restrict__ blk = cf + (int64_t)b * (4 * kCoefBlock);
    double t[kCoefBlock], mx = -INFINITY;
#pragma unroll
    for (int i = 0; i < kCoefBlock; ++i) {
      t[i] = b * kCoefBlock + i < K
                 ? fma(blk[2 * kCoefBlock + i], yn2, fma(blk[kCoefBlock + i], yn, blk[i]))
                 : -INFINITY;
      mx = fmax(mx, t[i]);
    }
    nlive += (unsigned)min(kCoefBlock, K - b * kCoefBlock);
    const double mn = fmax(a.m, ceil(mx));
    a.s = ldexp(a.s, (int)fmax(a.m - mn, -2100.0));
    a.m = mn;
    const double ms = mn == -INFINITY ? 0.0 : mn;
    double sum = 0.0;
#pragma unroll
    for (int i = 0; i < kCoefBlock; ++i) sum += exp2(t[i] - ms);
    a.s += sum;
  }
  acc[l][j] = a;
  if (census && j == 0 && nlive) atomicAdd(&live_n, nlive);
  TabAcc ce{-INFINITY, 0.0}, cg{-INFINITY, 0.0};
  if constexpr (LEAN) {
    const TabTerm *__restrict__ tt = terms + (int64_t)slot * kcap;
    for (int k = tid; k < K; k += 2 * kTabThreads) {
      const int k1 = k + kTabThreads;
      const TabTerm t0 = tt[k], t1 = tt[min(k1, K - 1)];
      double te0, tg0, te1, tg1;
      tab_cert_terms(t0, pl, ph, te0, tg0);
      tab_cert_terms(t1, pl, ph, te1, tg1);
      if (!(tab_add_noop(ce, te0) && tab_add_noop(cg, tg0))) {
        tab_add(ce, te0);
        tab_add(cg, tg0);
      }
      if (k1 < K && !(tab_add_noop(ce, te1) && tab_add_noop(cg, tg1))) {
        tab_add(ce, te1);
        tab_add(cg, tg1);
      }
    }
  } else {
    for (int k = tid; k < K; k += kTabThreads) {
      const double x = cf[coef_off(k, 0)], y = cf[coef_off(k, 1)], z = cf[coef_off(k, 2)];
      const double ak = -z, mu = y / (2.0 * ak), cc = x + ak * mu * mu;
      const double d = fmax(0.0, fmax(pl - mu, mu - ph)), df = fmax(mu - pl, ph - mu);
      tab_add(ce, cc + 8.0 * log2(2.0 * ak / L2E) - 0.5 * ak * d * d);
      tab_add(cg, cc - ak * df * df);
    }
  }
  ce = tab_wave_sum(ce);
  cg = tab_wave_sum(cg);
  if ((tid & 63) == 0) { cert[0][tid >> 6] = ce; cert[1][tid >> 6] = cg; }
  __syncthreads();
  double nm = -INFINITY, ns = 0.0;
  if (tid < kTabNodes) {
    TabAcc v = acc[0][tid];
    for (int q = 1; q < 16; ++q) tab_merge(v, acc[q][tid]);
    nm = v.m;
    ns = v.s;
    double M = nm;
#pragma unroll
    for (int o = 8; o > 0; o >>= 1) M = fmax(M, __shfl_xor(M, o, 64));
    fn[tid] = ldexp(ns, (int)fmax(nm - (M == -INFINITY ? 0.0 : M), -2100.0));
    if (tid == 0) red[0] = M;
  }
  __syncthreads();
  const double M = red[0];
  if (tid < kTabNodes) {
    double c = 0.0;
    for (int q = 0; q < kTabNodes; ++q)
      c = fma(fn[q], cospi((double)(tid * (2 * q + 1)) / 32.0), c);
    c *= tid == 0 ? 1.0 / 16.0 : 2.0 / 16.0;
    cn[tid] = c;
    tab[(int64_t)slot * kTabMaxPanels + p].c[tid] = c;
  }
  __syncthreads();
  if (tid != 0) return;
  tab[(int64_t)slot * kTabMaxPanels + p].M = M;
  tab[(int64_t)slot * kTabMaxPanels + p].pad = 0.0;
  if (census) {
    atomicAdd(census + 3, (unsigned long long)kTabNodes * (unsigned long long)K);
    atomicAdd(census + 5, (unsigned long long)kTabNodes * (unsigned long long)live_n);
  }
  bool ok = M > -INFINITY && M < INFINITY;
  double ca = 0.0;
  for (int q = 0; q < kTabNodes; ++q) {
    ok = ok && fn[q] > 0.0 && fn[q] < INFINITY;
    ca += fabs(cn[q]);
  }
  TabAcc E = cert[0][0], G = cert[1][0];
  for (int q = 1; q < 4; ++q) { tab_merge(E, cert[0][q]); tab_merge(G, cert[1][q]); }
  const double kL16 = 44.25014046988262;
  const double le = 0.11960158 + 0.5 * kL16 + (E.m + log2(E.s)) + 16.0 * log2(Hh) - 15.0 - kL16;
  const double lr = M + log2(ca) - 46.0;
  const double lg = G.m + log2(G.s);
  ok = ok && le == le && le < INFINITY && lg > -INFINITY && lg < INFINITY &&
       fmax(le, lr) + 1.0 <= lg - 28.0;
  if (ok) atomicAdd(&hdr[slot].ncert, 1u);
  if (cert_out) {
    double *c = cert_out + ((int64_t)slot * kTabMaxPanels + p) * 3;
    c[0] = le;
    c[1] = lr;
    c[2] = lg;
  }
}

__global__ __launch_bounds__(kTabThreads) void k_table_build(
    const tpe_hp *__restrict__ hps, const MixInfo *__restrict__ info,
    const Coef *__restrict__ coef, int64_t kcap, TabHdr *__restrict__ hdr,
    TabPanel *__restrict__ tab, unsigned long long *__restrict__ census,
    double *__restrict__ cert_out) {
  table_build_body<false>(hps, info, coef, kcap, hdr, tab, census, nullptr, nullptr, cert_out);
}
__global__ __launch_bounds__(kTabThreads) __attribute__((amdgpu_waves_per_eu(6)))
void k_table_build_lean(
    const tpe_hp *__restrict__ hps, const MixInfo *__restrict__ info,
    const Coef *__restrict__ coef, int64_t kcap, TabHdr *__restrict__ hdr,
    TabPanel *__restrict__ tab, unsigned long long *__restrict__ census,
    const TabTerm *__restrict__ terms, const double *__restrict__ a2s,
    double *__restrict__ cert_out) {
  table_build_body<true>(hps, info, coef, kcap, hdr, tab, census, terms, a2s, cert_out);
}

constexpr int kBndThreads = 256;
constexpr double kBndWiden = 0x1p-20;
constexpr int kBndPieces = 8;
static_assert(kBndCells % kBndThreads == 0 && kBndCells >= 2 * kTabMaxPanels, "lattice shape");

struct BndSide {
  double va, vb;
  double lo;
  double d1, d2;
  double e;
  double M;
};
__device__ __forceinline__ BndSide bound_side(const TabHdr &h, const TabPanel *__restrict__ tab,
                                              double xa, double xb) {
  const double um = (0.5 * (xa + xb) - h.y_lo) * h.inv_w;
  const double pf = fmin(fmax(floor(um), 0.0), (double)(h.P - 1));
  const TabPanel &pn = tab[(int)pf];
  double c[kTabNodes];
#pragma unroll
  for (int k = 0; k < kTabNodes; ++k) c[k] = pn.c[k];
  const double ta = fmin(fmax(2.0 * ((xa - h.y_lo) * h.inv_w - pf) - 1.0, -1.0), 1.0);
  const double tb = fmin(fmax(2.0 * ((xb - h.y_lo) * h.inv_w - pf) - 1.0, -1.0), 1.0);
  double s0 = 0.0, s1 = 0.0, s2 = 0.0;
#pragma unroll
  for (int k = 0; k < kTabNodes; ++k) {
    const double a = fabs(c[k]), k2 = (double)(k * k);
    s0 += a;
    s1 += k2 * a;
    s2 += k2 * (k2 - 1.0) / 3.0 * a;
  }
  BndSide r;
  r.va = tab_clenshaw(c, ta);
  r.vb = tab_clenshaw(c, tb);
  r.d1 = s1 * (2.0 * h.inv_w);
  r.d2 = s2 * (4.0 * h.inv_w * h.inv_w);
  r.e = s0 * 0x1p-46 + s1 * 0x1p-40;
  const double hh = xb - xa;
  r.lo = fmin(r.va, r.vb) - hh * hh * 0.125 * r.d2 - r.e;
  r.M = pn.M;
  return r;
}
__device__ __forceinline__ double bound_next_edge(const TabHdr &h, double x) {
  const double w = 1.0 / h.inv_w;
  const double j = floor((x - h.y_lo) * h.inv_w) + 1.0;
  const double e = h.y_lo + j * w;
  return e > x ? e : h.y_lo + (j + 1.0) * w;
}

__global__ __launch_bounds__(kBndThreads) void k_table_bound(
    const tpe_hp *__restrict__ hps, const TabHdr *__restrict__ hdr,
    const TabPanel *__restrict__ tab, double *__restrict__ bound) {
  const int hp = blockIdx.y, cell = blockIdx.x * kBndThreads + threadIdx.x;
  const tpe_hp H = hps[hp];
  if (!table_hp(H)) return;
  const TabHdr hb = hdr[2 * (int64_t)hp], ha = hdr[2 * (int64_t)hp + 1];
  if (!(tab_valid(hb) && tab_valid(ha))) return;
  const TabPanel *__restrict__ tb = tab + 2 * (int64_t)hp * kTabMaxPanels;
  const TabPanel *__restrict__ ta = tb + kTabMaxPanels;
  const double LN2 = 0.6931471805599453;
  const double y_lo = H.low - H.prior_mu, y_hi = H.high - H.prior_mu;
  const double cw = (y_hi - y_lo) / (double)kBndCells;
  const double a0 = cell == 0 ? y_lo : fmax(y_lo, y_lo + cw * ((double)cell - kBndWiden));
  const double b0 =
      cell == kBndCells - 1 ? y_hi : fmin(y_hi, y_lo + cw * ((double)(cell + 1) + kBndWiden));
  double U = -INFINITY, x = a0;
  bool ok = a0 < b0;
  for (int it = 0; it < kBndPieces && ok && x < b0; ++it) {
    const double nx = fmin(b0, fmin(bound_next_edge(hb, x), bound_next_edge(ha, x)));
    const BndSide B = bound_side(hb, tb, x, nx), A = bound_side(ha, ta, x, nx);
    const double la = log2(B.va / A.va), lb = log2(B.vb / A.vb), dm = B.M - A.M;
    const double sa = (dm + la) * LN2, sb = (dm + lb) * LN2;
    const double gb = B.d1 / B.lo, ga = A.d1 / A.lo;
    const double curv = B.d2 / B.lo + gb * gb + A.d2 / A.lo + ga * ga;
    const double slack =
        2.0 * (B.e / B.lo + A.e / A.lo) + 0x1p-40 * (1.0 + fabs(dm) + fabs(la) + fabs(lb));
    const double hh = nx - x;
    const double u = fmax(sa, sb) + hh * hh * 0.125 * curv + slack;
    ok = B.lo > 0.0 && A.lo > 0.0 && sa == sa && sb == sb && u == u && u < INFINITY;
    U = fmax(U, u);
    x = nx;
  }
  ok = ok && !(x < b0);
  bound[(int64_t)hp * kBndCells + cell] = ok ? U : INFINITY;
}

static_assert(sizeof(TabTerm) == kTabTermDoubles * sizeof(double), "terms scratch");
hipError_t launch_table_build(const tpe_hp *hps, int32_t n_hp, const MixInfo *info,
                              const Coef *coef, int64_t kcap, TabHdr *hdr, TabPanel *tab,
                              unsigned long long *census, hipStream_t st, double *bound,
                              double *terms, double *cert) {
  if (n_hp <= 0) return hipSuccess;
  hipError_t e = hipMemsetAsync(hdr, 0, (size_t)2 * n_hp * sizeof(TabHdr), st);
  if (e != hipSuccess) return e;
  const dim3 gb(kTabMaxPanels, 2 * n_hp);
  if (terms) {
    TabTerm *tt = reinterpret_cast<TabTerm *>(terms);
    double *a2s = terms + (int64_t)2 * n_hp * kcap * kTabTermDoubles;
    k_table_terms<<<dim3((unsigned)((kcap + kTabThreads - 1) / kTabThreads), 2 * n_hp), kTabThreads,
                    0, st>>>(hps, info, coef, kcap, tt, a2s);
    k_table_build_lean<<<gb, kTabThreads, 0, st>>>(hps, info, coef, kcap, hdr, tab, census, tt, a2s,
                                                   cert);
  } else {
    k_table_build<<<gb, kTabThreads, 0, st>>>(hps, info, coef, kcap, hdr, tab, census, cert);
  }
  if (bound)
    k_table_bound<<<dim3(kBndCells / kBndThreads, n_hp), kBndThreads, 0, st>>>(hps, hdr, tab, bound);
  return hipGetLastError();
}

}
```

hyperopt_amd/csrc/tpe_level_plan.hpp:

```cpp
#pragma once
#include <algorithm>
#include <cstdint>
#include <utility>
#include <vector>

#include "tpe_internal.hpp"
#include "tpe_switches.hpp"

namespace tpe {

constexpr int64_t kSortedDrawMin = (int64_t)1 << 22;
constexpr int64_t kSmallSortMin = 2048;
constexpr int64_t kTileDrawMax = 4096;

inline int32_t active_bound(const std::vector<tpe_hp> &all, const std::vector<int32_t> &cond_parent,
                            const std::vector<int32_t> &cond_branch, const int32_t *hps, int b,
                            int e) {
  int32_t n = 0;
  std::vector<std::pair<int32_t, int32_t>> pb;
  for (int i = b; i < e; ++i) {
    const tpe_hp &x = all[hps[i]];
    if (x.cond_count == 0) { ++n; continue; }
    std::vector<std::pair<int32_t, int32_t>> mine;
    for (int c = 0; c < x.cond_count; ++c)
// ... 50 lines not shown
        L.table_slot |= (k == KIND_LSE_G || k == KIND_LSE_L) && table_hp(hps[hp]);
      }
      while (L.n_lat < n && (L.kinds[L.n_lat] == KIND_ERF_G || L.kinds[L.n_lat] == KIND_ERF_L) &&
             lat[hl[L.n_lat]].R > 0) {
        L.rmax = std::max<int64_t>(L.rmax, lat[hl[L.n_lat]].R);
        ++L.n_lat;
      }
      auto bound = [&](int b, int e) {
        return active_bound(hps, cond_parent, cond_branch, hl.data(), b, e);
      };
      L.rows_level = bound(0, n);
      L.rows_lead = bound(0, L.n_lat);
      L.rows_plain.assign(n, 0);
      L.rows_lat.assign(n, 0);
      for (int with_lat = 0; with_lat < 2; ++with_lat) {
        auto kind = [&](int i) { return with_lat && i < L.n_lat ? (int)KIND_LAT : L.kinds[i]; };
        for (int j = 0; j < n;) {
          int k = j;
          while (k < n && kind(k) == kind(j)) ++k;
          (with_lat ? L.rows_lat : L.rows_plain)[j] = bound(j, k);
          j = k;
        }
      }
    }
  }
};

enum { BELOW_FUSE = 0,
       BELOW_TABLE = 1,
       BELOW_LARGE = 2 };
inline int below_class(int64_t k) {
  return k <= kFuseTab ? BELOW_FUSE : k <= kTabCap ? BELOW_TABLE : BELOW_LARGE;
}

struct FitVariant {
  bool small = false;
  int32_t mom_w = 0;
  bool mom_h = false;
  bool operator==(const FitVariant &o) const {
    return small == o.small && mom_w == o.mom_w && mom_h == o.mom_h;
  }
};

inline int32_t mom_width(const PlanShape &ps, const Switches &sw, int64_t n_hist) {
  if (!sw.moment) return 0;
  double kmax = 0.0;
  for (size_t i = 0; i < ps.hps.size(); ++i) {
    const int k = score_kind(ps.hps[i]);
    if (k == KIND_LSE_G || k == KIND_LSE_L) kmax = std::max(kmax, (double)n_hist * ps.act_frac[i]);
  }
  if (kmax >= (double)kMom16MinK) return 16;
  if (kmax >= (double)sw.lse_shift_min) return 8;
  return 0;
}

inline bool step_reads_moments(const PlanShape &ps, int64_t n_sug, int64_t n_cand) {
  bool sorted = false;
  for (const auto &l : ps.levels) sorted |= n_cand * n_sug * (int64_t)l.size() >= kSortedDrawMin;
  return sorted && n_cand > kWaveRowSplitMax;
}

inline FitVariant fit_variant(const PlanShape &ps, const Switches &sw, int64_t n_hist, bool small,
                              bool moments) {
  FitVariant f;
  f.small = small;
  f.mom_w = moments ? mom_width(ps, sw, n_hist) : 0;
  f.mom_h = f.mom_w == 16;
  return f;
}

struct StepShape {
  int64_t n_sug = 0, n_cand = 0, cand_begin = 0;
  int64_t n_total = 0;
  int32_t below = BELOW_LARGE;
  FitVariant fit;
  int32_t prune_mode = 3;
  bool lattice_on = true;
  bool capturing = false;
  bool publish = false;
  int32_t screen_run = 0;
  int32_t screen_halves = (int32_t)kDrawScreenHalves, screen_tail = (int32_t)kDrawScreenTail;
  bool screen_pool = false;
  bool table_lean = true;
  bool operator==(const StepShape &o) const {
    return n_sug == o.n_sug && n_cand == o.n_cand && cand_begin == o.cand_begin &&
           n_total == o.n_total && below == o.below && fit == o.fit &&
           prune_mode == o.prune_mode && lattice_on == o.lattice_on &&
           capturing == o.capturing && publish == o.publish && screen_run == o.screen_run &&
           screen_halves == o.screen_halves && screen_tail == o.screen_tail &&
           screen_pool == o.screen_pool && table_lean == o.table_lean;
  }
};
inline int32_t step_screen_run(const Switches &sw) {
  return sw.draw_screen && sw.draw_screen_int ? (int32_t)sw.draw_screen_run : 0;
}

inline int32_t step_screen_halves(const Switches &sw) {
  return sw.draw_screen_whole ? -1 : (int32_t)sw.draw_screen_halves;
}

struct ScoreGrid {
  int32_t n_groups = 0, pstride = 1;
  int32_t grp_kind[kMaxGroups] = {}, grp_slot0[kMaxGroups] = {}, grp_tiles[kMaxGroups] = {};
  int32_t grp_block0[kMaxGroups + 1] = {}, grp_slots[kMaxGroups] = {};
  int32_t blocks() const { return grp_block0[n_groups]; }
};
template <typename Kind, typename Rows>
ScoreGrid score_grid(Kind kind, int n_slots, int64_t cn, Rows rows) {
  ScoreGrid g;
  int32_t blocks = 0;
  auto weight = [](int k) {
    if (k == KIND_ERF_G || k == KIND_ERF_L) return 0;
    if (kind_lse(k)) return 1;
    return k == KIND_LAT ? 2 : 3;
  };
  for (int pass = 0; pass < 4; ++pass) {
    for (int j = 0; j < n_slots;) {
      int k = j;
      while (k < n_slots && kind(k) == kind(j)) ++k;
      if (weight(kind(j)) != pass) { j = k; continue; }
      if (g.n_groups == kMaxGroups) { g.pstride = -1; return g; }
      const int i = g.n_groups++;
      const int64_t tc = tile_cands(kind(j));
      const int32_t nt = (int32_t)((std::max<int64_t>(cn, 0) + tc - 1) / tc);
      g.grp_kind[i] = kind(j);
      g.grp_slot0[i] = j;
      g.grp_slots[i] = k - j;
      g.grp_tiles[i] = nt;
      g.grp_block0[i] = blocks;
      blocks += nt * std::min<int32_t>(k - j, rows(j, k));
      g.pstride = std::max(g.pstride, nt);
      j = k;
    }
  }
  g.grp_block0[g.n_groups] = blocks;
  return g;
}

inline int grid_classes(const ScoreGrid &g, bool lookup_draw) {
  int m = 0;
  for (int i = 0; i < g.n_groups; ++i) {
    const int k = g.grp_kind[i];
    m |= 1 << (kind_wave_lse(k) ? 0 : lookup_draw && (k == KIND_CAT || k == KIND_LAT) ? 1 : 2);
  }
  return m;
}

enum class LatRun {
  None,
  InOrder,
  Side,
  Deferred,
  Fused,
};

enum class Draw {
  Tiles,
  Fused,
  Plain,
  Sorted,
  SortedPruned,
  SortedScreened,
};

struct ChunkPlan {
  int64_t c0 = 0, cn = 0;
  bool accumulate = false;
  ScoreGrid grid;
  int32_t sort_log2 = 0, lse_pos = 0, lse_prune = 0, lse_f32 = 0, lookup_draw = 0;
  bool lk_fork = false;
  Draw draw = Draw::Plain;
  bool table_draw = false;
  bool small_table = false;
  bool fast = false;
  int32_t screen_tiles = 0;
  int32_t screen_halves = 0;
  int32_t screen_tail = 128;
  bool screen_pool = false;
  int32_t screen_guide = -1;
  int32_t screen_run = 0;
  bool bucket = false;
  bool cand_pos = false;
  int32_t tab_on = 0, tab_pref = 0;
  int classes = 7;
  bool publish = false;
};

struct LevelPlan {
  bool empty = false;
  int32_t n_level = 0;
  int32_t n_lat = 0;
  int32_t lat_rows = 0;
  bool compact = false;
  int32_t slot_rows = 0;
  bool erf_level = false;
  LatRun lat = LatRun::None;
  int32_t lse_shift_min = 0;
  std::vector<ChunkPlan> chunks;
};

inline LevelPlan plan_level(const PlanShape &ps, const Switches &sw, const StepShape &s,
                            int level) {
  const LevelShape &L = ps.lv[level];
  const std::vector<int32_t> &hl = ps.levels[level];
  const int32_t n_level = (int32_t)hl.size();
  const int64_t n_sug = s.n_sug, n_cand = s.n_cand;
  LevelPlan lp;
  lp.n_level = n_level;
  lp.lse_shift_min = (int32_t)sw.lse_shift_min;
  if (n_cand == 0) {
    lp.empty = true;
    return lp;
  }
  const int below = std::max(s.below, below_class(L.cat_upper));
  const bool table_draw = below <= BELOW_TABLE, small_table = below == BELOW_FUSE;
  const bool lat_level = L.n_lat > 0 && s.lattice_on && L.rmax <= n_cand * n_sug &&
                         2 * ((ps.kcap + 15) / 16) <= (int64_t)kLatChunks;
  const int32_t n_lat = lat_level ? L.n_lat : 0;
  lp.n_lat = n_lat;
  bool has_other = false;
  for (int i = n_lat; i < n_level; ++i) {
    lp.erf_level |= L.kinds[i] == KIND_ERF_G || L.kinds[i] == KIND_ERF_L;
    has_other |= L.kinds[i] != KIND_CAT;
  }
  lp.compact = L.rows_level < n_level;
  lp.slot_rows = lp.compact ? L.rows_level : n_level;
  lp.lat_rows = lp.compact && n_lat > 0
                    ? (int32_t)std::min<int64_t>(n_lat, n_sug * (int64_t)L.rows_lead)
                    : n_lat;
  auto rows = [&](int b, int e) {
    return lp.compact ? (lat_level ? L.rows_lat : L.rows_plain)[b] : e - b;
  };
  int64_t chunk = std::max<int64_t>(
      1, std::min<int64_t>(n_cand, sw.chunk_budget() / std::max<int64_t>(1, n_sug * n_level)));
  if (chunk < n_cand) chunk = std::max<int64_t>(kSortedBlock, chunk / kSortedBlock * kSortedBlock);
  auto sorted_size = [&](int64_t cn) { return cn * n_sug * n_level >= kSortedDrawMin; };
  const bool fuse_draw = lat_level && n_lat <= kLatJobs && small_table && chunk >= n_cand &&
                         !sorted_size(n_cand);
  const bool lookup_inline = small_table && !s.capturing && sw.lookup_draw;
  const bool lat_defer = lat_level && !fuse_draw && !sw.side_streams && has_other &&
                         table_draw && sorted_size(std::min(chunk, n_cand)) && lookup_inline &&
                         sw.lookup_fork;
  lp.lat = !lat_level ? LatRun::None
           : fuse_draw ? LatRun::Fused
           : lat_defer ? LatRun::Deferred
           : sw.side_streams ? LatRun::Side : LatRun::InOrder;
  int64_t lse_slots = 0;
  for (int j = 0; j < n_level;) {
    int k = j;
    while (k < n_level && L.kinds[k] == L.kinds[j]) ++k;
    if (j >= n_lat && (L.kinds[j] == KIND_LSE_G || L.kinds[j] == KIND_LSE_L))
      lse_slots += rows(j, k);
    j = k;
  }
  const bool one_row = lse_slots > 0 && n_sug * lse_slots * ((n_cand + 127) / 128) < 3 * kNumCUs;
  const bool wave1 = s.n_total <= kWaveRowSplitMax;

  for (int64_t c0 = 0; c0 < n_cand; c0 += chunk) {
    ChunkPlan c;
    c.c0 = c0;
    c.cn = std::min(chunk, n_cand - c0);
    c.accumulate = c0 > 0;
    c.table_draw = table_draw;
    c.small_table = small_table;
    const bool sorted = !fuse_draw && table_draw && sorted_size(c.cn);
    const bool small_sort = !sorted && sw.small_sort && c.cn >= kSmallSortMin && lse_slots > 0;
    const bool wave = sorted && s.prune_mode > 1;
    auto kind = [&](int i) -> int {
      if (i < n_lat) return KIND_LAT;
      const int k = L.kinds[i];
      if (k != KIND_LSE_G && k != KIND_LSE_L) return k;
      const bool lg = k == KIND_LSE_L;
      if (wave) return wave1 ? (lg ? KIND_LSE_LW1 : KIND_LSE_GW1) : (lg ? KIND_LSE_LW : KIND_LSE_GW);
      return one_row || small_sort ? (lg ? KIND_LSE_L1 : KIND_LSE_G1) : k;
    };
    c.grid = score_grid(kind, n_level, c.cn, rows);
    c.lse_pos = sorted || small_sort ? 1 : 0;
    c.sort_log2 = sort_log2_for(s.n_total);
    c.lookup_draw = sorted && lookup_inline ? 1 : 0;
    c.lse_prune = sorted || small_sort ? s.prune_mode : 0;
    c.lse_f32 = s.prune_mode == 3 ? 1 : 0;
    c.tab_on = L.table_slot && wave && !wave1 && s.prune_mode == 3 && s.fit.mom_w == 16 && sw.table
                   ? 1 : 0;
    c.tab_pref = c.tab_on && sw.table_prefilter ? 1 : 0;
    const int cls = grid_classes(c.grid, c.lookup_draw != 0);
    c.lk_fork = (cls & 2) && (cls & ~2) && sw.lookup_fork;
    c.classes = c.lk_fork ? 5 : 7;
    const bool tdraw = !sorted && !small_sort && !fuse_draw && !lat_level && !lp.erf_level &&
                       small_table && c.cn <= kTileDrawMax && !s.capturing && sw.tile_draw;
    c.publish = tdraw && s.publish && level + 1 == (int)ps.levels.size() && c.cn == n_cand &&
                s.cand_begin == 0 && s.n_total == n_cand && !lp.compact && !c.lk_fork &&
                c.grid.n_groups > 0 && c.grid.blocks() > 0 && sw.publish_fuse;
    if (tdraw) {
      c.draw = Draw::Tiles;
    } else if (fuse_draw) {
      c.draw = Draw::Fused;
    } else if (sorted) {
      c.fast = true;
      for (int i = 0; i < n_level && c.fast; ++i) {
        const tpe_hp &x = ps.hps[hl[i]];
        const bool lookup = i < n_lat || L.kinds[i] == KIND_CAT;
        c.fast = lookup ? c.lookup_draw != 0
                        : (x.family != TPE_CAT && (x.flags & TPE_HAS_LOW) && (x.flags & TPE_HAS_HIGH));
      }
      const bool prune = c.tab_on == 1 && c.tab_pref && (cls & 1) && sw.draw_prune &&
                         c.sort_log2 == kSortLog2Large && c.cn > kSortedBlock;
      const bool screen = prune && c.fast && small_table && sw.draw_screen &&
                          c.cn * n_sug * n_level >= sw.draw_screen_min;
      c.draw = screen ? Draw::SortedScreened : prune ? Draw::SortedPruned : Draw::Sorted;
      c.screen_tiles = (int32_t)sw.draw_screen_tiles;
      c.screen_halves = s.screen_halves;
      c.screen_tail = s.screen_tail;
      c.screen_pool = s.screen_pool;
      c.screen_guide = sw.draw_screen_int ? (int32_t)sw.draw_screen_guide_bits : -1;
      c.screen_run = screen && c.screen_guide >= 0 ? s.screen_run : 0;
      if (prune) c.tab_pref = 2;
    } else {
      c.draw = Draw::Plain;
    }
    c.bucket = (lp.erf_level || small_sort) && !sorted;
    c.cand_pos = lp.erf_level || sorted || small_sort;
    lp.chunks.push_back(c);
  }
  return lp;
}

}
```

hyperopt_amd/csrc/tpe_switches.hpp:

```cpp
#pragma once
#include <cmath>
#include <cstdint>
#include <cstdlib>

#include "tpe_internal.hpp"

namespace tpe {

struct Switches {
  bool lookup_draw;
  bool lookup_fork;
  bool publish;
  bool tile_draw;
  bool publish_fuse;
  bool moment;
  bool table;
  bool draw_prune;
  bool draw_screen;
  bool draw_screen_int;
  bool table_prefilter;
  bool table_scalar;
  bool table_lean;
  bool small_sort;
  bool side_streams;
  bool graph;
  int64_t table_tie_log2;
  int64_t draw_screen_tiles;
  bool draw_screen_whole;
  int64_t draw_screen_halves;
  int64_t draw_screen_tail;
  bool draw_screen_pool;
  int64_t draw_screen_min;
  int64_t draw_screen_guide_bits;
  int64_t draw_screen_run;
  int64_t chunk_mb;
  int64_t lse_shift_min;

  double table_tie() const { return std::ldexp(1.0, (int)table_tie_log2); }
  int64_t chunk_budget() const { return chunk_mb << 17; }
};

constexpr int64_t kDrawScreenMin = (int64_t)1 << 26;
constexpr int64_t kDrawScreenRun = 4;
constexpr int64_t kDrawScreenHalves = 4;
constexpr int64_t kDrawScreenTail = 24;

enum class SwitchRule {
  OffIfZero,
  OffIfNonEmptyZero,
  OnIfNonZero,
  OnIfSet,
  OnIfNonEmpty,
  ValueIfSet,
  ValueIfNonEmpty,
};

struct SwitchDef {
  const char *name;
  SwitchRule rule;
  int64_t dflt;
  bool Switches::*flag;
  int64_t Switches::*value;
  int64_t lo, hi;
};

constexpr int64_t kTabTieLog2 = -16;
static_assert(kTabTie == 0x1p-16, "kTabTie is 2^kTabTieLog2");

inline const SwitchDef *switch_table(int *n) {
  using R = SwitchRule;
  using S = Switches;
  constexpr int64_t lo = INT64_MIN, hi = INT64_MAX;
  static const SwitchDef defs[] = {
      {"TPE_LOOKUP_DRAW", R::OffIfZero, 1, &S::lookup_draw, nullptr, 0, 0},
      {"TPE_LOOKUP_FORK", R::OffIfZero, 1, &S::lookup_fork, nullptr, 0, 0},
      {"TPE_PUBLISH", R::OffIfZero, 1, &S::publish, nullptr, 0, 0},
      {"TPE_TILE_DRAW", R::OffIfZero, 1, &S::tile_draw, nullptr, 0, 0},
      {"TPE_PUBLISH_FUSE", R::OffIfZero, 1, &S::publish_fuse, nullptr, 0, 0},
      {"TPE_MOMENT", R::OffIfZero, 1, &S::moment, nullptr, 0, 0},
      {"TPE_TABLE", R::OffIfZero, 1, &S::table, nullptr, 0, 0},
      {"TPE_DRAW_PRUNE", R::OffIfNonEmptyZero, 1, &S::draw_prune, nullptr, 0, 0},
      {"TPE_DRAW_SCREEN", R::OffIfNonEmptyZero, 1, &S::draw_screen, nullptr, 0, 0},
      {"TPE_DRAW_SCREEN_INT", R::OffIfNonEmptyZero, 1, &S::draw_screen_int, nullptr, 0, 0},
      {"TPE_TABLE_PREFILTER", R::OffIfNonEmptyZero, 1, &S::table_prefilter, nullptr, 0, 0},
      {"TPE_TABLE_SCALAR", R::OffIfNonEmptyZero, 1, &S::table_scalar, nullptr, 0, 0},
      {"TPE_TABLE_LEAN", R::OffIfNonEmptyZero, 1, &S::table_lean, nullptr, 0, 0},
      {"TPE_SMALL_SORT", R::OnIfNonZero, 0, &S::small_sort, nullptr, 0, 0},
      {"TPE_SIDE_STREAMS", R::OnIfSet, 0, &S::side_streams, nullptr, 0, 0},
      {"TPE_GRAPH", R::OnIfSet, 0, &S::graph, nullptr, 0, 0},
      {"TPE_TABLE_TIE_LOG2", R::ValueIfSet, kTabTieLog2, nullptr, &S::table_tie_log2, -1074, 4096},
      {"TPE_DRAW_SCREEN_TILES", R::ValueIfNonEmpty, 2, nullptr, &S::draw_screen_tiles, 0,
       kPilotWaves},
      {"TPE_DRAW_SCREEN_TILES", R::OnIfNonEmpty, 0, &S::draw_screen_whole, nullptr, 0, 0},
      {"TPE_DRAW_SCREEN_HALVES", R::ValueIfNonEmpty, kDrawScreenHalves, nullptr,
       &S::draw_screen_halves, 0, 2 * kPilotWaves},
      {"TPE_DRAW_SCREEN_TAIL", R::ValueIfNonEmpty, kDrawScreenTail, nullptr, &S::draw_screen_tail, 1,
       128},
      {"TPE_DRAW_SCREEN_POOL", R::OnIfNonZero, 0, &S::draw_screen_pool, nullptr, 0, 0},
      {"TPE_DRAW_SCREEN_MIN", R::ValueIfNonEmpty, kDrawScreenMin, nullptr, &S::draw_screen_min, lo,
       hi},
      {"TPE_DRAW_SCREEN_GUIDE_BITS", R::ValueIfNonEmpty, 9, nullptr, &S::draw_screen_guide_bits, 0,
       kGuideBitsMax},
      {"TPE_DRAW_SCREEN_RUN", R::ValueIfNonEmpty, kDrawScreenRun, nullptr, &S::draw_screen_run, 0,
       kScreenRunMax},
      {"TPE_CHUNK_MB", R::ValueIfSet, 8192, nullptr, &S::chunk_mb, lo, hi},
      {"TPE_SHIFT_MIN_K", R::ValueIfSet, 512, nullptr, &S::lse_shift_min, lo, hi},
  };
  *n = (int)(sizeof(defs) / sizeof(defs[0]));
  return defs;
}

template <typename Get>
Switches read_switches(Get get) {
  Switches s{};
  int n = 0;
  const SwitchDef *defs = switch_table(&n);
  for (int i = 0; i < n; ++i) {
    const SwitchDef &d = defs[i];
    const char *e = get(d.name);
    switch (d.rule) {
      case SwitchRule::OffIfZero: s.*d.flag = !(e && std::atoi(e) == 0); break;
      case SwitchRule::OffIfNonEmptyZero: s.*d.flag = !(e && *e && std::atoi(e) == 0); break;
      case SwitchRule::OnIfNonZero: s.*d.flag = e && std::atoi(e) != 0; break;
      case SwitchRule::OnIfSet: s.*d.flag = e != nullptr; break;
      case SwitchRule::OnIfNonEmpty: s.*d.flag = e && *e; break;
      case SwitchRule::ValueIfSet:
      case SwitchRule::ValueIfNonEmpty: {
        const bool set = e && (d.rule == SwitchRule::ValueIfSet || *e);
        const int64_t v = set ? (int64_t)std::atoll(e) : d.dflt;
        s.*d.value = v < d.lo ? d.lo : v > d.hi ? d.hi : v;
        break;
      }
    }
  }
  return s;
}

inline const Switches &switches() {
  static const Switches s = read_switches([](const char *name) { return std::getenv(name); });
  return s;
}

}
```

include/tpe_engine.h:

```cpp
#ifndef TPE_ENGINE_H
#define TPE_ENGINE_H

#include <stdint.h>

#ifdef __cplusplus
extern "C" {
#endif

#define TPE_ENGINE_ABI_VERSION 1

#define TPE_SHARD_ALIGN 8192

#define TPE_OK 0
#define TPE_E_INVALID (-1)
#define TPE_E_BOUNDS (-2)
#define TPE_E_NEGATIVE (-3)
#define TPE_E_NOMEM (-4)
#define TPE_E_HIP (-5)
#define TPE_E_NODEVICE (-6)
#define TPE_E_INDEX (-7)

#define TPE_GMM 0
#define TPE_LGMM 1
#define TPE_CAT 2
// ... 137 lines not shown
                           int64_t ld, double *vals, double *total, double *terms,
                           uint8_t *active, int32_t on_device, void *stream);

int tpe_plan_topk_points(tpe_plan_t p, const double *total, const uint8_t *eligible,
                         int64_t m, int32_t k, int32_t *idx, int32_t on_device,
                         void *stream);

int tpe_plan_gather_points(tpe_plan_t p, const double *vals, int64_t ld,
                           const int32_t *idx, int32_t k, double *out,
                           int32_t on_device, void *stream);

int tpe_plan_joint_fit(tpe_plan_t p, void *stream);
int tpe_plan_joint_get_mixture(tpe_plan_t p, int32_t hp, int32_t side, double *w,
                               double *mu, double *sigma, int32_t *rows, int64_t cap,
                               int64_t *k);
int tpe_plan_joint_score_points(tpe_plan_t p, const double *vals, int64_t m, int64_t ld,
                                double *total, double *joint, double *terms,
                                uint8_t *active, int32_t on_device, void *stream);
int tpe_plan_joint_sides(tpe_plan_t p, double *below, double *above, int64_t m);
int tpe_plan_joint_sample_points(tpe_plan_t p, uint64_t seed, int64_t begin, int64_t m,
                                 int64_t ld, double *vals, int32_t *comp, double *total,
                                 double *joint, double *terms, uint8_t *active,
                                 int32_t on_device, void *stream);

int tpe_plan_group_info(tpe_plan_t p, int32_t *group_of_hp, int32_t *n_groups);
int tpe_plan_group_fit(tpe_plan_t p, void *stream);
int tpe_plan_group_get_mixture(tpe_plan_t p, int32_t group, int32_t hp, int32_t side,
                               double *w, double *mu, double *sigma, int32_t *rows,
                               int64_t cap, int64_t *k);
int tpe_plan_group_score_points(tpe_plan_t p, const double *vals, int64_t m, int64_t ld,
                                double *total, double *joint, uint8_t *active,
                                int32_t on_device, void *stream);
int tpe_plan_group_sides(tpe_plan_t p, int32_t group, double *below, double *above,
                         int64_t m);
int tpe_plan_group_sample_points(tpe_plan_t p, uint64_t seed, int64_t begin, int64_t m,
                                 int64_t ld, double *vals, int32_t *comp, double *total,
                                 double *joint, uint8_t *active, int32_t on_device,
                                 void *stream);

int tpe_plan_group_batch_points(tpe_plan_t p, const double *vals, int64_t m, int64_t ld,
                                const uint8_t *eligible, int32_t k, int32_t *idx,
                                double *gain, double *trace, int32_t on_device,
                                void *stream);

#define TPE_MAX_OBJ 8
int tpe_plan_set_objectives(tpe_plan_t p, const double *Y, int32_t n_obj, int64_t n,
                            int64_t ld, int64_t obj0, int32_t on_device, void *stream);

int tpe_plan_pareto_get(tpe_plan_t p, int32_t *dominated_by, int32_t *dominates,
                        double *loss, int64_t n);

int tpe_plan_pareto_shape(tpe_plan_t p, int64_t n, int32_t n_obj, int64_t force_splits,
                          int64_t *out);

int tpe_plan_set_hv(tpe_plan_t p, int32_t mode, const double *ref, int32_t n_obj,
                    int32_t n_pick, int32_t n_samples, uint64_t seed, int32_t method);

int tpe_plan_hv_get(tpe_plan_t p, int32_t *picks, double *keys, int32_t *counts,
                    int32_t *n_picked, int32_t cap);

int tpe_plan_last_stats(tpe_plan_t p, double *score_ms, double *pairs);

int tpe_plan_profile(tpe_plan_t p, int32_t capacity);
int tpe_plan_profile_read(tpe_plan_t p, int32_t kind, double *avg_ms,
                          int64_t *launches, double *pairs_per_launch);

int tpe_plan_set_lattice(tpe_plan_t p, int32_t enable);

int tpe_plan_census(tpe_plan_t p, int32_t enable, int64_t *counts);
int tpe_plan_census_n(tpe_plan_t p, int32_t enable, int64_t *counts, int32_t n_counts);

int tpe_plan_tie_counts(tpe_plan_t p, int32_t n_suggest, int32_t *counts);
int tpe_plan_tab_wmax(tpe_plan_t p, int32_t n_suggest, double *out);
int tpe_plan_tab_bound(tpe_plan_t p, int32_t hp, double *out);
int tpe_plan_tab_panels(tpe_plan_t p, int32_t hp, int32_t side, double *y_lo, double *inv_w,
                        int32_t *ncert, void *panels);
int tpe_plan_tab_cert(tpe_plan_t p, int32_t hp, int32_t side, double *out);
int tpe_plan_tie_list(tpe_plan_t p, int32_t s, int32_t hp, int32_t *out);
int tpe_plan_tab_hot(tpe_plan_t p, int32_t n_suggest, double *out);
int64_t tpe_plan_cand_dump(tpe_plan_t p, int32_t s, int32_t hp, double *values,
                           int32_t *positions);
int tpe_plan_draw_screen_stats(tpe_plan_t p, int64_t *out);

int tpe_plan_sample_prior(tpe_plan_t p, const uint64_t *seeds, int64_t n_suggest,
                          tpe_result *out, int32_t out_on_device, void *stream);

int tpe_plan_set_anneal_order(tpe_plan_t p, const int32_t *hp_order, int32_t n_hp);
int tpe_plan_anneal(tpe_plan_t p, double avg_best_idx, double shrink_coef,
                    const uint64_t *seeds, int64_t n_suggest,
                    tpe_result *out, int32_t out_on_device, void *stream);

typedef struct { int32_t row; int32_t rank; double u[4]; } tpe_anneal_trace;
int tpe_plan_anneal_trace(tpe_plan_t p, int32_t n_suggest, tpe_anneal_trace *out);

int tpe_plan_set_prune(tpe_plan_t p, int32_t mode);

int tpe_microbench(tpe_handle_t h, int32_t which, double *per_second);

int tpe_math_probe(tpe_handle_t h, int32_t which, const double *x, int64_t n, double *out);

#ifdef __cplusplus
}
#endif
#endif
```

Baseline: 1332000 billion pairs/s.

## Split single-level slots into groups pipelined across auxiliary streams

For single-level plans with large candidate counts, the hyperparameter slots are partitioned into up to four groups. Each group runs its fit, table build, draw and score on its own stream, with events chaining the draw phases so one group's scoring can overlap another's fit and draw. Fit, table-build and bound kernels gain an hp_list indirection so they can operate on a subset of slots. This adds event and launch overhead and more complex stream ordering, in exchange for hiding serial phase latency.

```diff
diff --git a/hyperopt_amd/_engine.py b/hyperopt_amd/_engine.py
--- a/hyperopt_amd/_engine.py
+++ b/hyperopt_amd/_engine.py
@@ -37,7 +37,8 @@
     'tpe_plan_tie_counts', 'tpe_plan_tab_wmax', 'tpe_plan_anneal', 'tpe_plan_anneal_trace',
     'tpe_plan_set_anneal_order', 'tpe_plan_tab_bound', 'tpe_plan_tab_hot',
     'tpe_plan_tab_panels', 'tpe_plan_tab_cert', 'tpe_plan_tie_list',
-    'tpe_plan_cand_dump', 'tpe_plan_draw_screen_stats', 'tpe_plan_score_points',
+    'tpe_plan_cand_dump', 'tpe_plan_draw_screen_stats', 'tpe_plan_slot_groups',
+    'tpe_plan_score_points',
     'tpe_plan_sample_points', 'tpe_plan_topk_points', 'tpe_plan_gather_points',
     'tpe_plan_joint_fit', 'tpe_plan_joint_get_mixture', 'tpe_plan_joint_score_points',
     'tpe_plan_joint_sides', 'tpe_plan_joint_sample_points', 'tpe_math_probe',
@@ -189,6 +190,7 @@
             'tpe_plan_tie_list': (C.c_int, [vp, i32, i32, vp]),
             'tpe_plan_cand_dump': (C.c_int64, [vp, i32, i32, vp, vp]),
             'tpe_plan_draw_screen_stats': (C.c_int, [vp, vp]),
+            'tpe_plan_slot_groups': (C.c_int, [vp, vp, vp]),
             'tpe_plan_set_lattice': (C.c_int, [vp, i32]),
             'tpe_plan_set_prune': (C.c_int, [vp, i32]),
             'tpe_plan_sample_prior': (C.c_int, [vp, C.POINTER(u64), i64, vp, i32, vp]),
@@ -1096,6 +1098,15 @@
             e.check(e.lib.tpe_plan_draw_screen_stats(self.p, out.ctypes.data))
         return int(out[0]), int(out[1]), int(out[2])
 
+    def slot_groups(self):
+        e = self.engine
+        n = np.zeros(1, dtype=np.int32)
+        s0 = np.zeros(5, dtype=np.int32)
+        with e.lock:
+            e.check(e.lib.tpe_plan_slot_groups(self.p, n.ctypes.data, s0.ctypes.data))
+        g = int(n[0])
+        return g, [(int(s0[i]), int(s0[i + 1])) for i in range(g)]
+
     def last_stats(self):
         e = self.engine
         ms, pairs = C.c_double(0), C.c_double(0)
diff --git a/hyperopt_amd/csrc/tpe_engine.hip b/hyperopt_amd/csrc/tpe_engine.hip
--- a/hyperopt_amd/csrc/tpe_engine.hip
+++ b/hyperopt_amd/csrc/tpe_engine.hip
@@ -87,6 +87,8 @@
   bool lattice_on = true;
   int32_t prune_mode = 3;
   hipEvent_t ev_fork = nullptr, ev_join[8] = {};
+  hipEvent_t ev_grp[3 * (kMaxSlotGroups - 1)] = {};
+  SlotGroups last_groups;
   double *d_ext = nullptr, *d_lb = nullptr, *d_la = nullptr;
   size_t ext_cap = 0;
   double *d_pt_vals = nullptr, *d_pt_terms = nullptr, *d_pt_total = nullptr;
@@ -284,6 +286,7 @@
   if (p->ev1) (void)hipEventDestroy(p->ev1);
   if (p->ev_fork) (void)hipEventDestroy(p->ev_fork);
   for (auto e : p->ev_join) if (e) (void)hipEventDestroy(e);
+  for (auto e : p->ev_grp) if (e) (void)hipEventDestroy(e);
   for (auto &pr : p->prof) {
     for (auto e : pr.a) (void)hipEventDestroy(e);
     for (auto e : pr.b) (void)hipEventDestroy(e);
@@ -460,6 +463,7 @@
   CKH(hipEventCreate(&p->ev1));
   CKH(hipEventCreateWithFlags(&p->ev_fork, hipEventDisableTiming));
   for (auto &e : p->ev_join) CKH(hipEventCreateWithFlags(&e, hipEventDisableTiming));
+  for (auto &e : p->ev_grp) CKH(hipEventCreateWithFlags(&e, hipEventDisableTiming));
   std::vector<int32_t> lh;
   for (auto &l : p->levels) lh.insert(lh.end(), l.begin(), l.end());
   std::vector<int32_t> all(p->P);
@@ -739,11 +743,132 @@
   s.screen_tail = (int32_t)switches().draw_screen_tail;
   s.screen_pool = switches().draw_screen_pool;
   s.table_lean = switches().table_lean;
+  s.instrumented = p->prof_cap > 0 || p->census;
   return s;
 }
 
-int run_level(tpe_engine *h, tpe_plan *p, int level, const StepShape &s, hipStream_t st) {
+struct StepFit {
+  int32_t nb;
+  double prior_weight;
+  int32_t lf;
+};
+
+int run_level_groups(tpe_engine *h, tpe_plan *p, int level, const StepShape &s, hipStream_t st,
+                     const LevelPlan &lp, const SlotGroups &sg, const StepFit *fit) {
+  const ChunkPlan &c = lp.chunks[0];
+  const int64_t n_sug = s.n_sug, cn = c.cn;
+  const int32_t n_level = lp.n_level;
+  const int32_t *lvl = p->d_level_hps + p->level_off[level];
+  int rc = ensure_suggest_state(h, p, n_sug, (size_t)n_sug * p->P * c.grid.pstride);
+  if (rc) return rc;
+  rc = ensure_cand(h, p, (size_t)std::max<int64_t>(1, n_sug * n_level * cn));
+  if (rc) return rc;
+  FitArgs fa{};
+  const HistPatch *patch = nullptr;
+  if (fit) {
+    fa = fit_args(p, fit->nb, fit->prior_weight, fit->lf, s.fit);
+    patch = p->has_pend ? &p->pend : nullptr;
+  }
+  const bool build = !p->tab_built;
+  if (build)
+    CKH(hipMemsetAsync(p->d_tab_hdr, 0, (size_t)2 * p->P * sizeof(TabHdr), st));
+  auto stream_of = [&](int g) { return g == 0 ? st : h->aux[g - 1]; };
+  auto ev = [&](int g, int k) { return p->ev_grp[3 * (g - 1) + k]; };
+  int forked = 0;
+  auto groups = [&]() -> int {
+    for (int g = 0; g < sg.n; ++g) {
+      hipStream_t sq = stream_of(g);
+      const int32_t b = sg.slot0[g], ns = sg.slot0[g + 1] - b;
+      if (g > 0) {
+        CKH(hipStreamWaitEvent(sq, ev(g, 0), 0));
+        forked = g;
+      }
+      if (fit) {
+        FitArgs ga = fa;
+        ga.hp_list = lvl + b;
+        CKH(launch_fit(ga, ns, sq, patch));
+      }
+      if (build)
+        CKH(launch_table_build(p->d_hps, p->P, p->d_info, p->d_coef, p->kcap, p->d_tab_hdr, p->d_tab,
+                               nullptr, sq, switches().table_prefilter ? p->d_tab_bound : nullptr,
+                               p->d_tab_terms, p->d_tab_cert, lvl + b, ns));
+      ScoreArgs a = base_args(p, n_sug);
+      copy_groups(a, slice_grid(c.grid, b, b + ns));
+      a.compact = 0;
+      a.cand = p->d_cand + (int64_t)b * cn;
+      int32_t *cpos = p->d_cpos + (int64_t)b * cn;
+      a.cand_sstride = (int64_t)n_level * cn;
+      a.n_cand = cn;
+      a.cand_begin = s.cand_begin + c.c0;
+      a.accumulate = 0;
+      a.level_hps = lvl + b;
+      a.n_slots = ns;
+      a.slot_rows = ns;
+      a.cand_slot0 = 0;
+      for (int i = 0; i < kInlineSeeds && i < n_sug; ++i) a.seed_inline[i] = p->h_seeds[i];
+      a.n_inline_seeds = (int32_t)std::min<int64_t>(n_sug, kInlineSeeds);
+      a.lse_pos = c.lse_pos;
+      a.sort_log2 = c.sort_log2;
+      a.lookup_draw = c.lookup_draw;
+      a.lse_prune = c.lse_prune;
+      a.lse_shift_min = lp.lse_shift_min;
+      a.lse_f32 = c.lse_f32;
+      a.tab_on = c.tab_on;
+      a.tab_pref = c.tab_pref ? 1 : 0;
+      a.tile_draw = 0;
+      CKH(launch_draw_sorted(a, c.small_table, c.fast, cpos, sq, 1, lp.slot_rows));
+      CKH(launch_table_pilot(a, sq));
+      if (c.draw == Draw::SortedScreened)
+        CKH(launch_draw_zone(a, p->d_draw_zone, c.screen_tiles, c.screen_halves, c.screen_tail,
+                             kScreenMargin, c.screen_guide, sq));
+      if (g + 1 < sg.n) CKH(hipEventRecord(ev(g + 1, 0), sq));
+      if (g > 0) CKH(hipStreamWaitEvent(sq, ev(g, 1), 0));
+      if (c.draw == Draw::SortedScreened)
+        CKH(launch_draw_screened(a, cpos, p->d_draw_zone, p->d_screen_stats, c.screen_guide >= 0,
+                                 c.screen_run, c.screen_pool, sq));
+      else
+        CKH(launch_draw_pruned(a, c.small_table, c.fast, cpos, sq));
+      if (g + 1 < sg.n) CKH(hipEventRecord(ev(g + 1, 1), sq));
+      a.tab_pref = c.tab_pref;
+      a.cand_pos = c.cand_pos ? cpos : nullptr;
+      CKH(launch_score(a, lp.erf_level, sq, nullptr, nullptr, nullptr, c.classes));
+    }
+    return TPE_OK;
+  };
+  rc = groups();
+  bool joined = true;
+  for (int g = 1; g <= forked; ++g) {
+    const hipError_t e1 = hipEventRecord(ev(g, 2), stream_of(g));
+    joined = joined && e1 == hipSuccess &&
+             hipStreamWaitEvent(st, ev(g, 2), 0) == hipSuccess;
+  }
+  if (fit) {
+    p->has_pend = false;
+    p->last_nb = fit->nb;
+  }
+  if (rc) return rc;
+  if (!joined) return fail(h, TPE_E_HIP, "join of the slot group streams");
+  if (build) p->tab_built = true;
+  p->tab_pstride = c.grid.pstride;
+  p->dump_cn = cn;
+  p->dump_sstride = (int64_t)n_level * cn;
+  p->dump_level = level;
+  p->dump_nsug = n_sug;
+  return TPE_OK;
+}
+
+int run_level(tpe_engine *h, tpe_plan *p, int level, const StepShape &s, hipStream_t st,
+              const StepFit *fit = nullptr) {
   const LevelPlan lp = plan_level(*p, switches(), s, level);
+  const SlotGroups sg = plan_slot_groups(lp, s, switches());
+  p->last_groups = sg;
+  if (sg.n > 1) return run_level_groups(h, p, level, s, st, lp, sg, fit);
+  if (fit) {
+    const int rc =
+        fit_launch(h, p, fit_args(p, fit->nb, fit->prior_weight, fit->lf, s.fit), p->P, st);
+    if (rc) return rc;
+    p->last_nb = fit->nb;
+  }
   const int64_t n_sug = s.n_sug;
   const int32_t n_level = lp.n_level, n_lat = lp.n_lat;
   const int32_t *lvl = p->d_level_hps + p->level_off[level];
@@ -1726,6 +1851,10 @@
 
 int enqueue_step(tpe_engine *h, tpe_plan *p, int32_t nb, double prior_weight, int32_t lf,
                  const StepShape &s, hipStream_t st) {
+  if (p->levels.size() == 1) {
+    const StepFit f{nb, prior_weight, lf};
+    return run_level(h, p, 0, s, st, &f);
+  }
   {
     const int rc = fit_launch(h, p, fit_args(p, nb, prior_weight, lf, s.fit), p->P, st);
     if (rc) return rc;
@@ -3302,6 +3431,14 @@
   return n;
 }
 
+int tpe_plan_slot_groups(tpe_plan_t p, int32_t *n_groups, int32_t *slot0) {
+  if (!p || !n_groups || !slot0) return TPE_E_INVALID;
+  *n_groups = p->last_groups.n;
+  for (int g = 0; g <= kMaxSlotGroups; ++g)
+    slot0[g] = p->last_groups.slot0[std::min<int>(g, p->last_groups.n)];
+  return TPE_OK;
+}
+
 int tpe_plan_draw_screen_stats(tpe_plan_t p, int64_t *out) {
   if (!p || !out) return TPE_E_INVALID;
   tpe_engine *h = p->eng;
diff --git a/hyperopt_amd/csrc/tpe_fit.hip b/hyperopt_amd/csrc/tpe_fit.hip
--- a/hyperopt_amd/csrc/tpe_fit.hip
+++ b/hyperopt_amd/csrc/tpe_fit.hip
@@ -969,7 +969,7 @@
   extern __shared__ __attribute__((aligned(16))) unsigned char dyn_lds[];
   __shared__ FitShared sm;
   if (P.n_rows > 0 || P.n_loss > 0) {
-    const int hp = blockIdx.x;
+    const int hp = A.hp_list ? A.hp_list[blockIdx.x] : (int)blockIdx.x;
     double *vals = const_cast<double *>(A.vals);
     uint8_t *act = const_cast<uint8_t *>(A.active);
     double *losses = const_cast<double *>(A.losses);
@@ -990,7 +990,7 @@
 template <bool SMALL>
 __device__ __forceinline__ void fit_slot(const FitArgs &A, unsigned char *dyn_lds,
                                          FitShared &sm) {
-  const int hp = blockIdx.x, side = blockIdx.y;
+  const int hp = A.hp_list ? A.hp_list[blockIdx.x] : (int)blockIdx.x, side = blockIdx.y;
   const int64_t slot = 2 * (int64_t)hp + side;
   const tpe_hp H = A.hps[hp];
   FitCtx C;
diff --git a/hyperopt_amd/csrc/tpe_internal.hpp b/hyperopt_amd/csrc/tpe_internal.hpp
--- a/hyperopt_amd/csrc/tpe_internal.hpp
+++ b/hyperopt_amd/csrc/tpe_internal.hpp
@@ -275,6 +275,7 @@
   double *tmp;
   unsigned char *sortbuf;
   int64_t scap;
+  const int32_t *hp_list;
 };
 
 hipError_t launch_split(const FitArgs &a, uint8_t *below, hipStream_t st);
@@ -328,7 +329,8 @@
   return n_total > kWaveRowSplitMax ? kSortLog2Large : kSortLog2Small;
 }
 hipError_t launch_draw_sorted(const ScoreArgs &a, bool small_table, bool fast, int32_t *pos_out,
-                              hipStream_t st, int64_t max_blocks = INT64_MAX);
+                              hipStream_t st, int64_t max_blocks = INT64_MAX,
+                              int32_t width_rows = 0);
 hipError_t launch_draw_pruned(const ScoreArgs &a, bool small_table, bool fast, int32_t *pos_out,
                               hipStream_t st);
 constexpr int kZoneMax = 6;
@@ -381,7 +383,8 @@
 hipError_t launch_table_build(const tpe_hp *hps, int32_t n_hp, const MixInfo *info,
                               const Coef *coef, int64_t kcap, TabHdr *hdr, TabPanel *tab,
                               unsigned long long *census, hipStream_t st, double *bound = nullptr,
-                              double *terms = nullptr, double *cert = nullptr);
+                              double *terms = nullptr, double *cert = nullptr,
+                              const int32_t *hp_list = nullptr, int32_t n_list = 0);
 
 constexpr int kPatchVals = 192;
 constexpr int kPatchLoss = 16;
diff --git a/hyperopt_amd/csrc/tpe_kernels.hip b/hyperopt_amd/csrc/tpe_kernels.hip
--- a/hyperopt_amd/csrc/tpe_kernels.hip
+++ b/hyperopt_amd/csrc/tpe_kernels.hip
@@ -632,12 +632,13 @@
 }
 
 hipError_t launch_draw_sorted(const ScoreArgs &a, bool small_table, bool fast, int32_t *pos_out,
-                              hipStream_t st, int64_t max_blocks) {
+                              hipStream_t st, int64_t max_blocks, int32_t width_rows) {
   if (a.n_slots <= 0 || a.n_suggest <= 0 || a.n_cand <= 0) return hipSuccess;
   const int64_t sbk = (int64_t)1 << a.sort_log2;
   const unsigned gx = (unsigned)std::min<int64_t>((a.n_cand + sbk - 1) / sbk, max_blocks);
   const dim3 g(gx, (unsigned)a.slot_rows, a.n_suggest);
-  const bool wide = (int64_t)gx * a.slot_rows * a.n_suggest <= 2 * kNumCUs;
+  const bool wide =
+      (int64_t)gx * (width_rows > 0 ? width_rows : a.slot_rows) * a.n_suggest <= 2 * kNumCUs;
   if (wide) {
     if (fast) {
       if (small_table) k_draw_sorted_wide_fast<kFuseTab><<<g, kWideDrawThreads, 0, st>>>(a, pos_out);
@@ -755,11 +756,16 @@
 }
 #pragma clang fp contract(fast)
 
+__device__ __forceinline__ int table_list_slot(const int32_t *__restrict__ hp_list, unsigned y) {
+  return hp_list ? 2 * hp_list[y >> 1] + (int)(y & 1u) : (int)y;
+}
+
 __global__ __launch_bounds__(kTabThreads) void k_table_terms(
     const tpe_hp *__restrict__ hps, const MixInfo *__restrict__ info,
     const Coef *__restrict__ coef, int64_t kcap, TabTerm *__restrict__ terms,
-    double *__restrict__ a2s) {
-  const int slot = blockIdx.y, tid = threadIdx.x, k = blockIdx.x * kTabThreads + tid;
+    double *__restrict__ a2s, const int32_t *__restrict__ hp_list) {
+  const int slot = table_list_slot(hp_list, blockIdx.y), tid = threadIdx.x,
+            k = blockIdx.x * kTabThreads + tid;
   if (!table_hp(hps[slot >> 1])) return;
   const int K = info[slot].K;
   if (K < 1 || K > kcap) return;
@@ -790,8 +796,8 @@
     const Coef *__restrict__ coef, int64_t kcap, TabHdr *__restrict__ hdr,
     TabPanel *__restrict__ tab, unsigned long long *__restrict__ census,
     const TabTerm *__restrict__ terms, const double *__restrict__ a2s,
-    double *__restrict__ cert_out) {
-  const int slot = blockIdx.y, p = blockIdx.x, tid = threadIdx.x;
+    double *__restrict__ cert_out, const int32_t *__restrict__ hp_list) {
+  const int slot = table_list_slot(hp_list, blockIdx.y), p = blockIdx.x, tid = threadIdx.x;
   const tpe_hp H = hps[slot >> 1];
   if (!table_hp(H)) return;
   const MixInfo mi = info[slot];
@@ -958,8 +964,9 @@
     const tpe_hp *__restrict__ hps, const MixInfo *__restrict__ info,
     const Coef *__restrict__ coef, int64_t kcap, TabHdr *__restrict__ hdr,
     TabPanel *__restrict__ tab, unsigned long long *__restrict__ census,
-    double *__restrict__ cert_out) {
-  table_build_body<false>(hps, info, coef, kcap, hdr, tab, census, nullptr, nullptr, cert_out);
+    double *__restrict__ cert_out, const int32_t *__restrict__ hp_list) {
+  table_build_body<false>(hps, info, coef, kcap, hdr, tab, census, nullptr, nullptr, cert_out,
+                          hp_list);
 }
 __global__ __launch_bounds__(kTabThreads) __attribute__((amdgpu_waves_per_eu(6)))
 void k_table_build_lean(
@@ -967,8 +974,8 @@
     const Coef *__restrict__ coef, int64_t kcap, TabHdr *__restrict__ hdr,
     TabPanel *__restrict__ tab, unsigned long long *__restrict__ census,
     const TabTerm *__restrict__ terms, const double *__restrict__ a2s,
-    double *__restrict__ cert_out) {
-  table_build_body<true>(hps, info, coef, kcap, hdr, tab, census, terms, a2s, cert_out);
+    double *__restrict__ cert_out, const int32_t *__restrict__ hp_list) {
+  table_build_body<true>(hps, info, coef, kcap, hdr, tab, census, terms, a2s, cert_out, hp_list);
 }
 
 constexpr int kBndThreads = 256;
@@ -1021,8 +1028,10 @@
 
 __global__ __launch_bounds__(kBndThreads) void k_table_bound(
     const tpe_hp *__restrict__ hps, const TabHdr *__restrict__ hdr,
-    const TabPanel *__restrict__ tab, double *__restrict__ bound) {
-  const int hp = blockIdx.y, cell = blockIdx.x * kBndThreads + threadIdx.x;
+    const TabPanel *__restrict__ tab, double *__restrict__ bound,
+    const int32_t *__restrict__ hp_list) {
+  const int hp = hp_list ? hp_list[blockIdx.y] : (int)blockIdx.y,
+            cell = blockIdx.x * kBndThreads + threadIdx.x;
   const tpe_hp H = hps[hp];
   if (!table_hp(H)) return;
   const TabHdr hb = hdr[2 * (int64_t)hp], ha = hdr[2 * (int64_t)hp + 1];
@@ -1060,24 +1069,30 @@
 hipError_t launch_table_build(const tpe_hp *hps, int32_t n_hp, const MixInfo *info,
                               const Coef *coef, int64_t kcap, TabHdr *hdr, TabPanel *tab,
                               unsigned long long *census, hipStream_t st, double *bound,
-                              double *terms, double *cert) {
-  if (n_hp <= 0) return hipSuccess;
-  hipError_t e = hipMemsetAsync(hdr, 0, (size_t)2 * n_hp * sizeof(TabHdr), st);
-  if (e != hipSuccess) return e;
-  const dim3 gb(kTabMaxPanels, 2 * n_hp);
+                              double *terms, double *cert, const int32_t *hp_list,
+                              int32_t n_list) {
+  if (n_hp <= 0 || (hp_list && n_list <= 0)) return hipSuccess;
+  if (!hp_list) {
+    const hipError_t e = hipMemsetAsync(hdr, 0, (size_t)2 * n_hp * sizeof(TabHdr), st);
+    if (e != hipSuccess) return e;
+  }
+  const int32_t rows = hp_list ? n_list : n_hp;
+  const dim3 gb(kTabMaxPanels, 2 * rows);
   if (terms) {
     TabTerm *tt = reinterpret_cast<TabTerm *>(terms);
     double *a2s = terms + (int64_t)2 * n_hp * kcap * kTabTermDoubles;
-    k_table_terms<<<dim3((unsigned)((kcap + kTabThreads - 1) / kTabThreads), 2 * n_hp), kTabThreads,
-                    0, st>>>(hps, info, coef, kcap, tt, a2s);
+    k_table_terms<<<dim3((unsigned)((kcap + kTabThreads - 1) / kTabThreads), 2 * rows), kTabThreads,
+                    0, st>>>(hps, info, coef, kcap, tt, a2s, hp_list);
     k_table_build_lean<<<gb, kTabThreads, 0, st>>>(hps, info, coef, kcap, hdr, tab, census, tt, a2s,
-                                                   cert);
+                                                   cert, hp_list);
   } else {
-    k_table_build<<<gb, kTabThreads, 0, st>>>(hps, info, coef, kcap, hdr, tab, census, cert);
+    k_table_build<<<gb, kTabThreads, 0, st>>>(hps, info, coef, kcap, hdr, tab, census, cert,
+                                              hp_list);
   }
   if (bound)
-    k_table_bound<<<dim3(kBndCells / kBndThreads, n_hp), kBndThreads, 0, st>>>(hps, hdr, tab, bound);
-  return hipGetLastError();
-}
-
-}
+    k_table_bound<<<dim3(kBndCells / kBndThreads, rows), kBndThreads, 0, st>>>(hps, hdr, tab, bound,
+                                                                               hp_list);
+  return hipGetLastError();
+}
+
+}
diff --git a/hyperopt_amd/csrc/tpe_level_plan.hpp b/hyperopt_amd/csrc/tpe_level_plan.hpp
--- a/hyperopt_amd/csrc/tpe_level_plan.hpp
+++ b/hyperopt_amd/csrc/tpe_level_plan.hpp
@@ -156,13 +156,15 @@
   int32_t screen_halves = (int32_t)kDrawScreenHalves, screen_tail = (int32_t)kDrawScreenTail;
   bool screen_pool = false;
   bool table_lean = true;
+  bool instrumented = false;
   bool operator==(const StepShape &o) const {
     return n_sug == o.n_sug && n_cand == o.n_cand && cand_begin == o.cand_begin &&
            n_total == o.n_total && below == o.below && fit == o.fit &&
            prune_mode == o.prune_mode && lattice_on == o.lattice_on &&
            capturing == o.capturing && publish == o.publish && screen_run == o.screen_run &&
            screen_halves == o.screen_halves && screen_tail == o.screen_tail &&
-           screen_pool == o.screen_pool && table_lean == o.table_lean;
+           screen_pool == o.screen_pool && table_lean == o.table_lean &&
+           instrumented == o.instrumented;
   }
 };
 inline int32_t step_screen_run(const Switches &sw) {
@@ -262,6 +264,7 @@
 
 struct LevelPlan {
   bool empty = false;
+  int32_t n_levels = 0;
   int32_t n_level = 0;
   int32_t n_lat = 0;
   int32_t lat_rows = 0;
@@ -280,6 +283,7 @@
   const int32_t n_level = (int32_t)hl.size();
   const int64_t n_sug = s.n_sug, n_cand = s.n_cand;
   LevelPlan lp;
+  lp.n_levels = (int32_t)ps.levels.size();
   lp.n_level = n_level;
   lp.lse_shift_min = (int32_t)sw.lse_shift_min;
   if (n_cand == 0) {
@@ -399,4 +403,57 @@
   return lp;
 }
 
-}
+struct SlotGroups {
+  int32_t n = 1;
+  int32_t slot0[kMaxSlotGroups + 1] = {};
+  bool operator==(const SlotGroups &o) const {
+    if (n != o.n) return false;
+    for (int g = 0; g <= n; ++g)
+      if (slot0[g] != o.slot0[g]) return false;
+    return true;
+  }
+};
+
+inline SlotGroups split_slots(int32_t n_slots, int32_t g) {
+  SlotGroups r;
+  r.n = std::max(1, std::min(g, n_slots));
+  const int32_t q = n_slots / r.n, rem = n_slots % r.n;
+  for (int i = 0; i < r.n; ++i) r.slot0[i + 1] = r.slot0[i] + q + (i < rem ? 1 : 0);
+  return r;
+}
+
+inline SlotGroups plan_slot_groups(const LevelPlan &lp, const StepShape &s, const Switches &sw) {
+  const SlotGroups one = split_slots(lp.n_level, 1);
+  if (sw.slot_groups <= 1 || lp.n_levels != 1 || lp.empty || lp.compact) return one;
+  if (lp.lat != LatRun::None || lp.n_lat != 0 || lp.chunks.size() != 1) return one;
+  if (s.capturing || sw.graph || s.instrumented) return one;
+  const ChunkPlan &c = lp.chunks[0];
+  if (c.draw != Draw::SortedScreened && c.draw != Draw::SortedPruned) return one;
+  if (c.lk_fork || c.publish || c.accumulate || c.bucket || c.grid.pstride < 0) return one;
+  if (grid_classes(c.grid, c.lookup_draw != 0) != 1) return one;
+  if (c.cn * s.n_sug * (int64_t)lp.n_level < sw.slot_groups_min) return one;
+  const int32_t g = (int32_t)std::min<int64_t>(
+      std::min<int64_t>(sw.slot_groups, kMaxSlotGroups), lp.n_level / 2);
+  return g <= 1 ? one : split_slots(lp.n_level, g);
+}
+
+inline ScoreGrid slice_grid(const ScoreGrid &g, int32_t b, int32_t e) {
+  ScoreGrid r;
+  r.pstride = g.pstride;
+  int32_t blocks = 0;
+  for (int i = 0; i < g.n_groups; ++i) {
+    const int32_t lo = std::max(g.grp_slot0[i], b), hi = std::min(g.grp_slot0[i] + g.grp_slots[i], e);
+    if (lo >= hi) continue;
+    const int j = r.n_groups++;
+    r.grp_kind[j] = g.grp_kind[i];
+    r.grp_slot0[j] = lo - b;
+    r.grp_slots[j] = hi - lo;
+    r.grp_tiles[j] = g.grp_tiles[i];
+    r.grp_block0[j] = blocks;
+    blocks += g.grp_tiles[i] * (hi - lo);
+  }
+  r.grp_block0[r.n_groups] = blocks;
+  return r;
+}
+
+}
diff --git a/hyperopt_amd/csrc/tpe_switches.hpp b/hyperopt_amd/csrc/tpe_switches.hpp
--- a/hyperopt_amd/csrc/tpe_switches.hpp
+++ b/hyperopt_amd/csrc/tpe_switches.hpp
@@ -33,6 +33,8 @@
   int64_t draw_screen_min;
   int64_t draw_screen_guide_bits;
   int64_t draw_screen_run;
+  int64_t slot_groups;
+  int64_t slot_groups_min;
   int64_t chunk_mb;
   int64_t lse_shift_min;
 
@@ -44,6 +46,9 @@
 constexpr int64_t kDrawScreenRun = 4;
 constexpr int64_t kDrawScreenHalves = 4;
 constexpr int64_t kDrawScreenTail = 24;
+constexpr int kMaxSlotGroups = 4;
+constexpr int64_t kSlotGroups = 4;
+constexpr int64_t kSlotGroupsMin = (int64_t)1 << 26;
 
 enum class SwitchRule {
   OffIfZero,
@@ -103,6 +108,10 @@
        kGuideBitsMax},
       {"TPE_DRAW_SCREEN_RUN", R::ValueIfNonEmpty, kDrawScreenRun, nullptr, &S::draw_screen_run, 0,
        kScreenRunMax},
+      {"TPE_SLOT_GROUPS", R::ValueIfNonEmpty, kSlotGroups, nullptr, &S::slot_groups, 1,
+       kMaxSlotGroups},
+      {"TPE_SLOT_GROUPS_MIN", R::ValueIfNonEmpty, kSlotGroupsMin, nullptr, &S::slot_groups_min, lo,
+       hi},
       {"TPE_CHUNK_MB", R::ValueIfSet, 8192, nullptr, &S::chunk_mb, lo, hi},
       {"TPE_SHIFT_MIN_K", R::ValueIfSet, 512, nullptr, &S::lse_shift_min, lo, hi},
   };
diff --git a/include/tpe_engine.h b/include/tpe_engine.h
--- a/include/tpe_engine.h
+++ b/include/tpe_engine.h
@@ -243,6 +243,8 @@
                            int32_t *positions);
 int tpe_plan_draw_screen_stats(tpe_plan_t p, int64_t *out);
 
+int tpe_plan_slot_groups(tpe_plan_t p, int32_t *n_groups, int32_t *slot0);
+
 int tpe_plan_sample_prior(tpe_plan_t p, const uint64_t *seeds, int64_t n_suggest,
                           tpe_result *out, int32_t out_on_device, void *stream);
 
```

New measurement: 1189000 billion pairs/s. 10.7% lower.
